# SparkJiao/llama-pipeline-parallel

Hardware: AMD Instinct MI355X
Metric: tokens/sec (whole node), LLaMA-65B PP=8 seq4096 at 1/2/4/8 MI355X (higher is better)
Workload: dtype bf16; 1 GPU; model=llama-65b, measured_model=llama-65b-shaped 10-layer slice (10/80 layers), global_batch=64, seq_len=4096, parallelism=pp1, num_layers=10, micro_batch_size=4, grad_accum_steps=16

## Files before the change

### lpp_amd/models/llama.py

```python

from __future__ import annotations

from typing import List, Optional

import torch
import torch.nn as nn

from ..config import ModelConfig
from ..layer_spec import LayerSpec
from .. import ops
from ..ops.linear import LPLinear, lp_linear


class RMSNorm(nn.Module):
    def __init__(self, hidden_size: int, eps: float = 1e-6):
        super().__init__()
        self.weight = nn.Parameter(torch.ones(hidden_size))
        self.variance_epsilon = eps

    def forward(self, x: torch.Tensor) -> torch.Tensor:
        return ops.rmsnorm(x, self.weight, self.variance_epsilon)


class KVCache:

    def __init__(self, batch: int, max_len: int, kv_heads: int, head_dim: int,
                 device, dtype):
        self.k = torch.zeros(batch, max_len, kv_heads, head_dim, device=device, dtype=dtype)
        self.v = torch.zeros_like(self.k)
        self.length = 0

    def append(self, k: torch.Tensor, v: torch.Tensor) -> int:
        S = k.shape[1]
        self.k[:, self.length : self.length + S] = k
        self.v[:, self.length : self.length + S] = v
        self.length += S
        return self.length


class SlotKVCache:

    def __init__(self, parent: "RaggedKVCache", slot: int):
        self.parent = parent
        self.slot = slot

    @property
    def k(self):
        return self.parent.k[self.slot : self.slot + 1]

    @property
    def v(self):
        return self.parent.v[self.slot : self.slot + 1]

    @property
    def length(self) -> int:
        return int(self.parent.lengths[self.slot])

    def append(self, k: torch.Tensor, v: torch.Tensor) -> int:
        S = k.shape[1]
        ln = self.length
        self.parent.k[self.slot, ln : ln + S] = k[0]
        self.parent.v[self.slot, ln : ln + S] = v[0]
        self.parent.lengths[self.slot] = ln + S
        return ln + S


class RaggedKVCache:

    per_row = True

    def __init__(self, slots: int, max_len: int, kv_heads: int, head_dim: int,
                 device, dtype):
        self.k = torch.zeros(slots, max_len, kv_heads, head_dim, device=device, dtype=dtype)
        self.v = torch.zeros_like(self.k)
        self.lengths = torch.zeros(slots, dtype=torch.long, device=device)

    def slot_view(self, slot: int) -> SlotKVCache:
        return SlotKVCache(self, slot)

    def free(self, slot: int) -> None:
        self.lengths[slot] = 0


class MultiSlotKVCache:

    def __init__(self, parent: RaggedKVCache, slots: torch.Tensor):
        self.parent = parent
        self.slots = slots
        self.length = 0

    def append(self, k: torch.Tensor, v: torch.Tensor) -> int:
        S = k.shape[1]
        self.parent.k[self.slots, self.length : self.length + S] = k
        self.parent.v[self.slots, self.length : self.length + S] = v
        self.length += S
        self.parent.lengths[self.slots] = self.length
        return self.length


class GatherKVCache:

    per_row = True

    def __init__(self, parent: RaggedKVCache, slots: torch.Tensor,
                 contiguous_range: Optional[tuple] = None,
                 total_hint: Optional[int] = None):
        self.parent = parent
        self.slots = slots
        self.range = contiguous_range
        self.total_hint = total_hint

    @property
    def k(self):
        return self.parent.k[self.slots]

    @property
    def v(self):
        return self.parent.v[self.slots]

    def kv_to(self, T: int):
        if self.range is not None:
            lo, hi = self.range
            return self.parent.k[lo:hi, :T], self.parent.v[lo:hi, :T]
        return self.parent.k[self.slots, :T], self.parent.v[self.slots, :T]

    @property
    def lengths(self) -> torch.Tensor:
        if self.range is not None:
            lo, hi = self.range
            return self.parent.lengths[lo:hi]
        return self.parent.lengths[self.slots]

    @property
    def rows(self) -> torch.Tensor:
        if getattr(self, "_rows", None) is None:
            if self.range is not None:
                lo, hi = self.range
                self._rows = torch.arange(lo, hi, device=self.parent.lengths.device)
            else:
                self._rows = self.slots
        return self._rows

    def append_one(self, k: torch.Tensor, v: torch.Tensor) -> torch.Tensor:
        lens = self.lengths
        if self.range is not None:
            lo, hi = self.range
            rows = torch.arange(lo, hi, device=lens.device)
        else:
            rows = self.slots
        self.parent.k[rows, lens] = k[:, 0]
        self.parent.v[rows, lens] = v[:, 0]
        new = lens + 1
        self.parent.lengths[rows] = new
        return new


class LlamaAttention(nn.Module):

    def __init__(self, cfg: ModelConfig):
        super().__init__()
        self.num_heads = cfg.num_heads
        self.num_kv_heads = cfg.kv_heads
        self.head_dim = cfg.head_dim
        self.hidden_size = cfg.hidden_size
        self.rope_theta = cfg.rope_theta
        self.max_seq_len = cfg.max_seq_len
        self.q_proj = LPLinear(cfg.hidden_size, self.num_heads * self.head_dim)
        self.k_proj = LPLinear(cfg.hidden_size, self.num_kv_heads * self.head_dim)
        self.v_proj = LPLinear(cfg.hidden_size, self.num_kv_heads * self.head_dim)
        self.o_proj = LPLinear(self.num_heads * self.head_dim, cfg.hidden_size)

    def forward(self, x: torch.Tensor, cache: Optional["KVCache"] = None) -> torch.Tensor:
        B, S, _ = x.shape
        q = self.q_proj(x).view(B, S, self.num_heads, self.head_dim)
        k = self.k_proj(x).view(B, S, self.num_kv_heads, self.head_dim)
        v = self.v_proj(x).view(B, S, self.num_kv_heads, self.head_dim)
        cos, sin = ops.build_rope_cache(
            self.max_seq_len, self.head_dim, self.rope_theta, x.device
        )
        if cache is not None and getattr(cache, "per_row", False):
            assert S == 1, "ragged cache is a single-token decode contract"
            tick = getattr(cache, "tick", None)
            if ops.decode_attention_hip_supported(q, self.num_kv_heads):
                parent = getattr(cache, "parent", cache)
                pos = getattr(tick, "pos", None)
                o = ops.decode_attention(
                    q, k, v, parent.k, parent.v, cos, sin,
                    pos if pos is not None else cache.lengths,
                    rows=cache.rows if parent is not cache else None,
                    lengths=parent.lengths,
                    max_len=getattr(cache, "total_hint", None))
                return self.o_proj(o.reshape(B, S, self.num_heads * self.head_dim))
            if tick is not None:
                q = ops.apply_rope_cs(q, tick.cos, tick.sin)
                k = ops.apply_rope_cs(k, tick.cos, tick.sin)
            else:
                lens = cache.lengths
                q = ops.apply_rope_positions(q, cos, sin, lens)
                k = ops.apply_rope_positions(k, cos, sin, lens)
            new_lens = cache.append_one(k, v)
            hint = getattr(cache, "total_hint", None)
            T = hint if hint is not None else int(new_lens.max())
            if hasattr(cache, "kv_to"):
                kc, vc = cache.kv_to(T)
            else:
                kc, vc = cache.k[:, :T], cache.v[:, :T]
            rep = self.num_heads // self.num_kv_heads
            qt = q.transpose(1, 2)
            kt = kc.transpose(1, 2)
            vt = vc.transpose(1, 2)
            if rep > 1:
                kt = kt.repeat_interleave(rep, dim=1)
                vt = vt.repeat_interleave(rep, dim=1)
            if tick is not None:
                mask = tick.mask
            else:
                mask = (torch.arange(T, device=x.device)[None, :]
                        < new_lens[:, None])[:, None, None, :]
            o = torch.nn.functional.scaled_dot_product_attention(
                qt, kt, vt, attn_mask=mask
            ).transpose(1, 2).contiguous()
            return self.o_proj(o.reshape(B, S, self.num_heads * self.head_dim))
        pos = cache.length if cache is not None else 0
        if (S == 1 and pos > 0 and isinstance(cache, KVCache)
                and ops.decode_attention_hip_supported(q, self.num_kv_heads)):
            o = ops.decode_attention(q, k, v, cache.k, cache.v, cos, sin, pos,
                                     max_len=pos + 1)
            cache.length = pos + 1
            return self.o_proj(o.reshape(B, S, self.num_heads * self.head_dim))
        q = ops.apply_rope(q, cos, sin, pos_offset=pos)
        k = ops.apply_rope(k, cos, sin, pos_offset=pos)
        if cache is None:
            o = ops.causal_attention(q, k, v)
        else:
            total = cache.append(k, v)
            if S == total:
                o = ops.causal_attention(q, k, v)
            else:
                kc = cache.k[:, :total]
                vc = cache.v[:, :total]
                rep = self.num_heads // self.num_kv_heads
                qt = q.transpose(1, 2)
                kt = kc.transpose(1, 2)
                vt = vc.transpose(1, 2)
                if rep > 1:
                    kt = kt.repeat_interleave(rep, dim=1)
                    vt = vt.repeat_interleave(rep, dim=1)
                mask = None
                if S > 1:
                    qpos = torch.arange(pos, total, device=x.device)
                    kpos = torch.arange(total, device=x.device)
                    mask = kpos[None, :] <= qpos[:, None]
                o = torch.nn.functional.scaled_dot_product_attention(
                    qt, kt, vt, attn_mask=mask
                ).transpose(1, 2).contiguous()
        return self.o_proj(o.reshape(B, S, self.num_heads * self.head_dim))


class LlamaMLP(nn.Module):
    def __init__(self, cfg: ModelConfig):
        super().__init__()
        self.gate_proj = LPLinear(cfg.hidden_size, cfg.intermediate_size)
        self.up_proj = LPLinear(cfg.hidden_size, cfg.intermediate_size)
        self.down_proj = LPLinear(cfg.intermediate_size, cfg.hidden_size)

    def forward(self, x: torch.Tensor) -> torch.Tensor:
        return self.down_proj(ops.swiglu(self.gate_proj(x), self.up_proj(x)))


class DecoderLayerPipe(nn.Module):

    def __init__(self, cfg: ModelConfig, activation_checkpointing: bool = False):
        super().__init__()
        self.self_attn = LlamaAttention(cfg)
        self.mlp = LlamaMLP(cfg)
        self.input_layernorm = RMSNorm(cfg.hidden_size, cfg.rms_norm_eps)
        self.post_attention_layernorm = RMSNorm(cfg.hidden_size, cfg.rms_norm_eps)
        self.activation_checkpointing = activation_checkpointing

    def _forward_impl(self, hidden: torch.Tensor,
                      cache: Optional[KVCache] = None) -> torch.Tensor:
        hidden = hidden + self.self_attn(self.input_layernorm(hidden), cache=cache)
        hidden = hidden + self.mlp(self.post_attention_layernorm(hidden))
        return hidden

    def forward(self, hidden: torch.Tensor,
                cache: Optional[KVCache] = None) -> torch.Tensor:
        if self.activation_checkpointing and self.training and hidden.requires_grad:
            return torch.utils.checkpoint.checkpoint(
                self._forward_impl, hidden, use_reentrant=False, preserve_rng_state=False
            )
        return self._forward_impl(hidden, cache=cache)

    @staticmethod
    def spec_param_count(cfg: ModelConfig, activation_checkpointing: bool = False) -> int:
        h, i = cfg.hidden_size, cfg.intermediate_size
        kv = cfg.kv_heads * cfg.head_dim
        return h * h * 2 + 2 * h * kv + 3 * h * i + 2 * h


class EmbeddingPipe(nn.Embedding):

    def __init__(self, vocab_size: int, hidden_size: int):
        super().__init__(vocab_size, hidden_size)

    def forward(self, input_ids: torch.Tensor) -> torch.Tensor:
        return super().forward(input_ids)

    @staticmethod
    def spec_param_count(vocab_size: int, hidden_size: int) -> int:
        return vocab_size * hidden_size


class NormPipe(RMSNorm):

    @staticmethod
    def spec_param_count(hidden_size: int, eps: float = 1e-6) -> int:
        return hidden_size


class LMHeadPipe(nn.Linear):

    def __init__(self, hidden_size: int, vocab_size: int):
        super().__init__(hidden_size, vocab_size, bias=False)

    def forward(self, x: torch.Tensor) -> torch.Tensor:
        return lp_linear(x, self.weight)

    @staticmethod
    def spec_param_count(hidden_size: int, vocab_size: int) -> int:
        return hidden_size * vocab_size


def loss_fn(logits: torch.Tensor, labels: torch.Tensor) -> torch.Tensor:
    return ops.shifted_cross_entropy(logits, labels)


def get_layers_from_config(
    cfg: ModelConfig, activation_checkpointing: bool = False,
    checkpoint_fn=None,
) -> List[LayerSpec]:
    if cfg.tie_word_embeddings:
        raise ValueError(
            "tie_word_embeddings=True is not supported: LLaMA checkpoints are "
            "untied and the reference (README.md:44-46) warns against tying "
            "under pipeline parallelism. Set it to False.")
    specs: List[LayerSpec] = [LayerSpec(EmbeddingPipe, cfg.vocab_size, cfg.hidden_size)]
    for i in range(cfg.num_layers):
        ck = checkpoint_fn(i) if checkpoint_fn is not None else activation_checkpointing
        specs.append(LayerSpec(DecoderLayerPipe, cfg, ck))
    specs.append(LayerSpec(NormPipe, cfg.hidden_size, cfg.rms_norm_eps))
    specs.append(LayerSpec(LMHeadPipe, cfg.hidden_size, cfg.vocab_size))
    return specs


@torch.no_grad()
def init_weights(module: nn.Module, cfg: ModelConfig, generator: Optional[torch.Generator] = None):
    std = cfg.initializer_range
    for m in module.modules():
        if isinstance(m, nn.Linear):
            m.weight.normal_(0.0, std, generator=generator)
            if m.bias is not None:
                m.bias.zero_()
        elif isinstance(m, nn.Embedding):
            m.weight.normal_(0.0, std, generator=generator)
        elif isinstance(m, RMSNorm):
            m.weight.fill_(1.0)


@torch.no_grad()
def deterministic_layer_init(layer: nn.Module, cfg: ModelConfig, seed: int, global_idx: int):
    g = torch.Generator().manual_seed(seed * 100003 + global_idx)
    std = cfg.initializer_range
    for name, p in sorted(layer.named_parameters()):
        if p.dim() >= 2:
            p.copy_(torch.empty(p.shape, dtype=torch.float32).normal_(0.0, std, generator=g).to(p.dtype))
        else:
            p.fill_(1.0) if "norm" in name or isinstance(layer, (RMSNorm,)) else p.zero_()
    for m in layer.modules():
        if isinstance(m, RMSNorm):
            m.weight.fill_(1.0)


def init_pipeline_weights(pipeline_module, cfg: ModelConfig, seed: int) -> None:
    for local_idx, layer in enumerate(pipeline_module.layers):
        deterministic_layer_init(layer, cfg, seed, pipeline_module.global_layer_index(local_idx))


def init_monolithic_weights(model: "LlamaForCausalLM", seed: int) -> None:
    for gidx, layer in enumerate(model.layers):
        deterministic_layer_init(layer, model.cfg, seed, gidx)


def layers_from_model(model: "LlamaForCausalLM") -> List[nn.Module]:
    return list(model.layers)


class LlamaForCausalLM(nn.Module):

    def __init__(self, cfg: ModelConfig, activation_checkpointing: bool = False):
        super().__init__()
        self.cfg = cfg
        self.layers = nn.ModuleList(
            [s.build() for s in get_layers_from_config(cfg, activation_checkpointing)]
        )

    def forward(self, input_ids: torch.Tensor) -> torch.Tensor:
        x = input_ids
        for layer in self.layers:
            x = layer(x)
        return x

    def compute_loss(self, input_ids: torch.Tensor, labels: torch.Tensor) -> torch.Tensor:
        return loss_fn(self.forward(input_ids), labels)

    @torch.no_grad()
    def generate(self, input_ids: torch.Tensor, max_new_tokens: int,
                 eos_token_id: Optional[int] = None,
                 temperature: float = 0.0,
                 generator: Optional[torch.Generator] = None) -> torch.Tensor:
        was_training = self.training
        self.eval()
        B, S0 = input_ids.shape
        dev = input_ids.device
        p = next(self.parameters())
        max_len = S0 + max_new_tokens
        caches = [
            KVCache(B, max_len, self.cfg.kv_heads, self.cfg.head_dim, dev, p.dtype)
            for _ in range(self.cfg.num_layers)
        ]

        def step(ids: torch.Tensor) -> torch.Tensor:
            x = ids
            li = 0
            for layer in self.layers:
                if isinstance(layer, DecoderLayerPipe):
                    x = layer(x, cache=caches[li])
                    li += 1
                else:
                    x = layer(x)
            return x[:, -1]

        out = input_ids
        logits = step(input_ids)
        finished = torch.zeros(B, dtype=torch.bool, device=dev)
        for _ in range(max_new_tokens):
            if temperature > 0:
                probs = torch.softmax(logits.float() / temperature, dim=-1)
                nxt = torch.multinomial(probs, 1, generator=generator).squeeze(-1)
            else:
                nxt = logits.argmax(dim=-1)
            if eos_token_id is not None:
                nxt = torch.where(finished, torch.full_like(nxt, eos_token_id), nxt)
                finished |= nxt == eos_token_id
            out = torch.cat([out, nxt[:, None]], dim=1)
            if eos_token_id is not None and bool(finished.all()):
                break
            logits = step(nxt[:, None])
        if was_training:
            self.train()
        return out
```

### lpp_amd/ops/__init__.py

```python

from __future__ import annotations

import os

import torch

_EXT = None
_EXT_ERR: str | None = "not loaded yet"


def _load_extension():
    global _EXT, _EXT_ERR
    if _EXT is not None:
        return _EXT
    try:
        from . import build as _build

        _EXT = _build.load_extension()
        _EXT_ERR = None
        if torch.cuda.is_available():
            _pin_wgrad_algos(_EXT)
    except Exception as e:
        _EXT = None
        _EXT_ERR = f"{type(e).__name__}: {e}"
    return _EXT


def _pin_wgrad_algos(ext) -> None:
    import json

    path = os.path.join(os.path.dirname(__file__), "wgrad_algos.json")
    if not os.path.exists(path):
        return
    try:
        data = json.load(open(path))
        for entry in data.get("shapes", []):
            ext.wgrad_set_algo(entry["T"], entry["in"], entry["out"], entry["index"],
                               entry.get("kind", 0))
    except Exception as e:
        import logging

        logging.getLogger(__name__).warning(
            "wgrad algo pinning skipped: %s", e)


def force_eager() -> bool:
    return os.environ.get("LPP_FORCE_EAGER", "0") == "1"


def extension():
    ext = _load_extension()
    if ext is None:
        raise RuntimeError(
            "lpp_amd HIP extension is required on GPU but failed to load: "
            f"{_EXT_ERR}. Build it with `python -m lpp_amd.ops.build` "
            "(or __graft_entry__.build())."
        )
    return ext


def use_hip(*tensors: torch.Tensor) -> bool:
    if force_eager():
        return False
    if not tensors or not tensors[0].is_cuda:
        return False
    return True


from .rmsnorm import rmsnorm
from .rope import (build_rope_cache, apply_rope, apply_rope_positions,
                   apply_rope_cs)
from .swiglu import swiglu
from .cross_entropy import shifted_cross_entropy
from .attention import (causal_attention, decode_attention,
                        decode_attention_ref, decode_attention_hip_supported)

__all__ = [
    "rmsnorm",
    "build_rope_cache",
    "apply_rope",
    "apply_rope_positions",
    "apply_rope_cs",
    "swiglu",
    "shifted_cross_entropy",
    "causal_attention",
    "decode_attention",
    "decode_attention_ref",
    "decode_attention_hip_supported",
    "extension",
    "use_hip",
    "force_eager",
]
```

### lpp_amd/ops/csrc/bindings.cpp

```cpp
#include <torch/extension.h>

#include <string>
#include <tuple>
#include <vector>

std::vector<at::Tensor> rmsnorm_fwd(at::Tensor x, at::Tensor weight, double eps);
std::vector<at::Tensor> rmsnorm_bwd(at::Tensor dy, at::Tensor x, at::Tensor weight,
                                    at::Tensor invrms);
at::Tensor rope_fwd(at::Tensor x, at::Tensor cos_t, at::Tensor sin_t, int64_t pos_offset);
at::Tensor rope_bwd(at::Tensor dy, at::Tensor cos_t, at::Tensor sin_t, int64_t pos_offset);
at::Tensor swiglu_fwd(at::Tensor gate, at::Tensor up);
std::vector<at::Tensor> swiglu_bwd(at::Tensor dy, at::Tensor gate, at::Tensor up);
std::vector<at::Tensor> cross_entropy_fwd(at::Tensor logits, at::Tensor labels);
at::Tensor cross_entropy_bwd(at::Tensor logits, at::Tensor labels, at::Tensor lse,
                             double scale);
std::vector<at::Tensor> attention_fwd(at::Tensor q, at::Tensor k, at::Tensor v);
std::vector<at::Tensor> attention_bwd(at::Tensor dO, at::Tensor q, at::Tensor k,
                                      at::Tensor v, at::Tensor o, at::Tensor lse2);
void attention_set_block_order(int64_t mode);
int64_t attention_get_block_order();
at::Tensor attention_block_order(int64_t kind, int64_t nblk, int64_t nheads, int64_t G,
                                 int64_t mode);
at::Tensor attention_lds_addresses(std::string pattern, int64_t shape, int64_t idx);
std::vector<double> attention_time_kernel(std::string kernel, at::Tensor dO, at::Tensor q,
                                          at::Tensor k, at::Tensor v, at::Tensor o,
                                          at::Tensor lse2, int64_t mode, int64_t G,
                                          int64_t warmup, int64_t reps);
at::Tensor attention_decode(at::Tensor q, at::Tensor k_new, at::Tensor v_new,
                            at::Tensor k_cache, at::Tensor v_cache, at::Tensor cos_t,
                            at::Tensor sin_t, c10::optional<at::Tensor> positions,
                            c10::optional<at::Tensor> rows,
                            c10::optional<at::Tensor> lengths, int64_t uniform_pos,
                            int64_t max_len, int64_t chunk);
int64_t attention_decode_chunk();
at::Tensor mfma_test_16x16x32(at::Tensor A, at::Tensor B);
void wgrad_f32_accum(at::Tensor x, at::Tensor dy, at::Tensor dw);
void wgrad_f32_accum_pre(at::Tensor xT, at::Tensor dyT, at::Tensor dw);
void wgrad_bf16d_pre(at::Tensor xT, at::Tensor dyT, at::Tensor out);
at::Tensor transpose2d(at::Tensor in);
void accum_bf16_f32(at::Tensor dst, at::Tensor src);
std::vector<std::tuple<int64_t, double, std::string>> wgrad_tune(int64_t T, int64_t in,
                                                                 int64_t out,
                                                                 int64_t reps,
                                                                 int64_t kind);
void wgrad_set_algo(int64_t T, int64_t in, int64_t out, int64_t index, int64_t kind);
std::tuple<int64_t, std::string> wgrad_current_algo(int64_t T, int64_t in, int64_t out,
                                                    int64_t kind);
at::Tensor mfma_test_32x32x16(at::Tensor A, at::Tensor B);
std::vector<at::Tensor> attn_tile_test_roundtrip(at::Tensor tile);
at::Tensor attn_tile_test_tr_fragments(at::Tensor tile, int64_t shape, int64_t nrows,
                                       int64_t buf);
at::Tensor attn_tile_test_pack_pair(at::Tensor x);
at::Tensor attn_tile_test_pack_frag16(at::Tensor x);
void fused_adamw(std::vector<at::Tensor> params, std::vector<at::Tensor> masters,
                 std::vector<at::Tensor> grads, std::vector<at::Tensor> exp_avg,
                 std::vector<at::Tensor> exp_avg_sq, double lr, double beta1, double beta2,
                 double eps, double weight_decay, double bias1, double bias2,
                 double grad_scale);

PYBIND11_MODULE(TORCH_EXTENSION_NAME, m) {
  m.doc() = "lpp_amd gfx950 (MI355X/CDNA4) kernels";
  m.def("rmsnorm_fwd", &rmsnorm_fwd, "RMSNorm forward (y, invrms)");
  m.def("rmsnorm_bwd", &rmsnorm_bwd, "RMSNorm backward (dx, dw)");
  m.def("rope_fwd", &rope_fwd, "RoPE forward");
  m.def("rope_bwd", &rope_bwd, "RoPE backward");
  m.def("swiglu_fwd", &swiglu_fwd, "SwiGLU forward");
  m.def("swiglu_bwd", &swiglu_bwd, "SwiGLU backward (dgate, dup)");
  m.def("cross_entropy_fwd", &cross_entropy_fwd, "fused CE forward (loss_sum, lse, count)");
  m.def("cross_entropy_bwd", &cross_entropy_bwd, "fused CE backward (dlogits)");
  m.def("fused_adamw", &fused_adamw, "fused mixed-precision AdamW");
  m.def("attention_fwd", &attention_fwd, "flash causal attention forward (O, LSE2)");
  m.def("attention_bwd", &attention_bwd, "flash causal attention backward (dQ, dK, dV)");
  m.def("attention_set_block_order", &attention_set_block_order,
        "attention block order: 0 = legacy, 1 = XCD-balanced heavy-first (default, "
        "LPP_ATTN_ORDER)", py::arg("mode"));
  m.def("attention_get_block_order", &attention_get_block_order, "current order mode");
  m.def("attention_block_order", &attention_block_order,
        "host: [n,2] int (blk, head) of linear block ids 0..n-1; kind 0 fwd/dQ, 1 dK/dV",
        py::arg("kind"), py::arg("nblk"), py::arg("nheads"), py::arg("G"), py::arg("mode"));
  m.def("attention_time_kernel", &attention_time_kernel,
        "hipEvent ms per launch of one attention kernel (fwd|dq|dkdv) under an explicit "
        "block order", py::arg("kernel"), py::arg("dO"), py::arg("q"), py::arg("k"),
        py::arg("v"), py::arg("o"), py::arg("lse2"), py::arg("mode"), py::arg("G") = 0,
        py::arg("warmup") = 3, py::arg("reps") = 20);
  m.def("attention_decode", &attention_decode,
        "fused single-token decode: RoPE + KV-cache write + GQA attention over keys 0..p of "
        "each row's cache row -> o [N,1,H,128]; chunk 0 = the compiled-in chunk size",
        py::arg("q"), py::arg("k_new"), py::arg("v_new"), py::arg("k_cache"),
        py::arg("v_cache"), py::arg("cos"), py::arg("sin"), py::arg("positions"),
        py::arg("rows"), py::arg("lengths"), py::arg("uniform_pos"), py::arg("max_len"),
        py::arg("chunk") = 0);
  m.def("attention_decode_chunk", &attention_decode_chunk,
        "keys per workgroup of attention_decode");
  m.def("wgrad_f32_accum", &wgrad_f32_accum, "dW_f32 += dY^T @ X (hipBLASLt, beta=1)");
  m.def("wgrad_f32_accum_pre", &wgrad_f32_accum_pre,
        "dW_f32 += dyT @ xT^T, pre-transposed k-contiguous operands (hipBLASLt, beta=1)");
  m.def("transpose2d", &transpose2d, "bf16/fp16 [R,C] -> [C,R] LDS-tiled transpose");
  m.def("wgrad_bf16d_pre", &wgrad_bf16d_pre,
        "bf16-D pre-transposed wgrad GEMM into a reusable scratch (beta 0)");
  m.def("accum_bf16_f32", &accum_bf16_f32, "dst_f32 += src_bf16 (vectorised)");
  m.def("wgrad_tune", &wgrad_tune,
        "exhaustive hipBLASLt solution sweep for a wgrad shape -> [(index, ms, name)]",
        py::arg("T"), py::arg("in_dim"), py::arg("out"), py::arg("reps"), py::arg("kind") = 0);
  m.def("wgrad_set_algo", &wgrad_set_algo, "pin a hipBLASLt solution index for a shape",
        py::arg("T"), py::arg("in_dim"), py::arg("out"), py::arg("index"), py::arg("kind") = 0);
  m.def("wgrad_current_algo", &wgrad_current_algo,
        "current (heuristic-picked) solution for a shape -> (index, name)",
        py::arg("T"), py::arg("in_dim"), py::arg("out"), py::arg("kind") = 0);
  m.def("mfma_test_16x16x32", &mfma_test_16x16x32, "MFMA layout validation");
  m.def("mfma_test_32x32x16", &mfma_test_32x32x16, "MFMA 32x32x16 layout validation");
  m.def("attn_tile_test_roundtrip", &attn_tile_test_roundtrip,
        "attn_tile.h dual-use image: int16 [64,128] -> (tile by row reads, transpose by "
        "transposed reads) from one LDS image");
  m.def("attn_tile_test_tr_fragments", &attn_tile_test_tr_fragments,
        "attn_tile.h transposed reads: int16 [64,128] -> int16 [16,64,8], the B-fragments "
        "of MFMA shape 32 (frag = dt*4+ks) or 16 (frag = dt*2+half) as the kernels read them",
        py::arg("tile"), py::arg("shape"), py::arg("nrows") = 64, py::arg("buf") = 0);
  m.def("attention_lds_addresses", &attention_lds_addresses,
        "host: int32 [64] per-lane LDS byte addresses of one access pattern (stage | row | "
        "tr) of MFMA shape 32 or 16", py::arg("pattern"), py::arg("shape"), py::arg("idx"));
  m.def("attn_tile_test_pack_pair", &attn_tile_test_pack_pair,
        "attn_tile.h pack_pair: fp32 [32,32] in C layout -> int32 [64,2,4] A-fragment words");
  m.def("attn_tile_test_pack_frag16", &attn_tile_test_pack_frag16,
        "attn_tile.h pack_frag16: fp32 [32,16] in C layout -> int32 [64,4] A-fragment words");
}
```

### lpp_amd/ops/csrc/rmsnorm.hip

```cpp
#include "common.h"

namespace lpp {

constexpr int BLOCK = 256;

template <typename T, int VEC>
__global__ void rmsnorm_fwd_kernel(const T* __restrict__ x, const float* __restrict__ w,
                                   T* __restrict__ y, float* __restrict__ invrms,
                                   int64_t n_rows, int H, float eps) {
  __shared__ float red[BLOCK / kWave];
  for (int64_t row = blockIdx.x; row < n_rows; row += gridDim.x) {
    const T* xr = x + row * H;
    T* yr = y + row * H;
    using PV = Pack<T, VEC>;
    float ss = 0.f;
    for (int i = threadIdx.x * VEC; i < H; i += BLOCK * VEC) {
      PV buf = *reinterpret_cast<const PV*>(xr + i);
#pragma unroll
      for (int v = 0; v < VEC; ++v) {
        float f = to_f32(buf.v[v]);
        ss += f * f;
      }
    }
    float total = block_reduce_sum<BLOCK>(ss, red);
    float inv = rsqrtf(total / (float)H + eps);
    if (threadIdx.x == 0) invrms[row] = inv;
    for (int i = threadIdx.x * VEC; i < H; i += BLOCK * VEC) {
      PV xin = *reinterpret_cast<const PV*>(xr + i);
      PV out;
#pragma unroll
      for (int v = 0; v < VEC; ++v)
        out.v[v] = from_f32<T>(to_f32(xin.v[v]) * inv * w[i + v]);
      *reinterpret_cast<PV*>(yr + i) = out;
    }
  }
}

template <typename T>
__global__ void rmsnorm_fwd_kernel_s(const T* __restrict__ x, const float* __restrict__ w,
                                     T* __restrict__ y, float* __restrict__ invrms,
                                     int64_t n_rows, int H, float eps) {
  __shared__ float red[BLOCK / kWave];
  for (int64_t row = blockIdx.x; row < n_rows; row += gridDim.x) {
    const T* xr = x + row * H;
    T* yr = y + row * H;
    float ss = 0.f;
    for (int i = threadIdx.x; i < H; i += BLOCK) {
      float f = to_f32(xr[i]);
      ss += f * f;
    }
    float total = block_reduce_sum<BLOCK>(ss, red);
    float inv = rsqrtf(total / (float)H + eps);
    if (threadIdx.x == 0) invrms[row] = inv;
    for (int i = threadIdx.x; i < H; i += BLOCK)
      yr[i] = from_f32<T>(to_f32(xr[i]) * inv * w[i]);
  }
}

template <typename T, int VEC, int N_IT>
__global__ void rmsnorm_bwd_kernel_v(const T* __restrict__ dy, const T* __restrict__ x,
                                     const float* __restrict__ w,
                                     const float* __restrict__ invrms, T* __restrict__ dx,
                                     float* __restrict__ dw_partial, int64_t n_rows,
                                     int H) {
  __shared__ float red[BLOCK / kWave];
  using PV = Pack<T, VEC>;
  alignas(16) float dwacc[N_IT][VEC];
  alignas(16) float wreg[N_IT][VEC];
#pragma unroll
  for (int it = 0; it < N_IT; ++it) {
    const int i = threadIdx.x * VEC + it * BLOCK * VEC;
    *reinterpret_cast<Pack<float, 4>*>(&wreg[it][0]) =
        *reinterpret_cast<const Pack<float, 4>*>(w + i);
    *reinterpret_cast<Pack<float, 4>*>(&wreg[it][4]) =
        *reinterpret_cast<const Pack<float, 4>*>(w + i + 4);
#pragma unroll
    for (int v = 0; v < VEC; ++v) dwacc[it][v] = 0.f;
  }

  for (int64_t row = blockIdx.x; row < n_rows; row += gridDim.x) {
    const T* dyr = dy + row * H;
    const T* xr = x + row * H;
    T* dxr = dx + row * H;
    const float inv = invrms[row];
    PV dybuf[N_IT], xbuf[N_IT];
    float dot = 0.f;
#pragma unroll
    for (int it = 0; it < N_IT; ++it) {
      const int i = threadIdx.x * VEC + it * BLOCK * VEC;
      dybuf[it] = *reinterpret_cast<const PV*>(dyr + i);
      xbuf[it] = *reinterpret_cast<const PV*>(xr + i);
#pragma unroll
      for (int v = 0; v < VEC; ++v)
        dot += to_f32(dybuf[it].v[v]) * wreg[it][v] * to_f32(xbuf[it].v[v]);
    }
    const float total = block_reduce_sum<BLOCK>(dot, red);
    const float k = total * inv * inv * inv / (float)H;
#pragma unroll
    for (int it = 0; it < N_IT; ++it) {
      const int i = threadIdx.x * VEC + it * BLOCK * VEC;
      PV out;
#pragma unroll
      for (int v = 0; v < VEC; ++v) {
        const float d = to_f32(dybuf[it].v[v]);
        const float xi = to_f32(xbuf[it].v[v]);
        out.v[v] = from_f32<T>(d * wreg[it][v] * inv - xi * k);
        dwacc[it][v] += d * xi * inv;
      }
      *reinterpret_cast<PV*>(dxr + i) = out;
    }
  }
  float* my = dw_partial + (int64_t)blockIdx.x * H;
#pragma unroll
  for (int it = 0; it < N_IT; ++it) {
    const int i = threadIdx.x * VEC + it * BLOCK * VEC;
    *reinterpret_cast<Pack<float, 4>*>(my + i) = *reinterpret_cast<Pack<float, 4>*>(&dwacc[it][0]);
    *reinterpret_cast<Pack<float, 4>*>(my + i + 4) = *reinterpret_cast<Pack<float, 4>*>(&dwacc[it][4]);
  }
}

template <typename T>
__global__ void rmsnorm_bwd_kernel(const T* __restrict__ dy, const T* __restrict__ x,
                                   const float* __restrict__ w,
                                   const float* __restrict__ invrms, T* __restrict__ dx,
                                   float* __restrict__ dw, int64_t n_rows, int H) {
  __shared__ float red[BLOCK / kWave];
  extern __shared__ __attribute__((aligned(16))) char smem[];
  float* dw_loc = reinterpret_cast<float*>(smem);
  for (int i = threadIdx.x; i < H; i += BLOCK) dw_loc[i] = 0.f;
  __syncthreads();

  for (int64_t row = blockIdx.x; row < n_rows; row += gridDim.x) {
    const T* dyr = dy + row * H;
    const T* xr = x + row * H;
    T* dxr = dx + row * H;
    const float inv = invrms[row];
    float dot = 0.f;
    for (int i = threadIdx.x; i < H; i += BLOCK) {
      float d = to_f32(dyr[i]);
      float xi = to_f32(xr[i]);
      dot += d * w[i] * xi;
      dw_loc[i] += d * xi * inv;
    }
    float total = block_reduce_sum<BLOCK>(dot, red);
    float k = total * inv * inv * inv / (float)H;
    for (int i = threadIdx.x; i < H; i += BLOCK) {
      float d = to_f32(dyr[i]);
      float xi = to_f32(xr[i]);
      dxr[i] = from_f32<T>(d * w[i] * inv - xi * k);
    }
  }
  __syncthreads();
  for (int i = threadIdx.x; i < H; i += BLOCK) atomicAdd(&dw[i], dw_loc[i]);
}

}

std::vector<at::Tensor> rmsnorm_fwd(at::Tensor x, at::Tensor weight, double eps) {
  TORCH_CHECK(x.is_cuda() && x.is_contiguous(), "rmsnorm_fwd: x must be contiguous on GPU");
  const int H = x.size(-1);
  const int64_t n_rows = x.numel() / H;
  auto y = at::empty_like(x);
  auto invrms = at::empty({n_rows}, x.options().dtype(at::kFloat));
  auto w32 = weight.to(at::kFloat).contiguous();
  auto stream = lpp::current_stream();
  const int grid = lpp::grid_for(n_rows, 1, 4096);
  LPP_DISPATCH_FLOAT(x.scalar_type(), "rmsnorm_fwd", [&] {
    constexpr int VEC = 16 / sizeof(scalar_t);
    if (H % VEC == 0) {
      hipLaunchKernelGGL((lpp::rmsnorm_fwd_kernel<scalar_t, VEC>), dim3(grid),
                         dim3(lpp::BLOCK), 0, stream, (const scalar_t*)x.data_ptr(),
                         w32.data_ptr<float>(), (scalar_t*)y.data_ptr(),
                         invrms.data_ptr<float>(), n_rows, H, (float)eps);
    } else {
      hipLaunchKernelGGL((lpp::rmsnorm_fwd_kernel_s<scalar_t>), dim3(grid),
                         dim3(lpp::BLOCK), 0, stream, (const scalar_t*)x.data_ptr(),
                         w32.data_ptr<float>(), (scalar_t*)y.data_ptr(),
                         invrms.data_ptr<float>(), n_rows, H, (float)eps);
    }
  });
  LPP_CHECK_HIP(hipGetLastError());
  return {y, invrms};
}

std::vector<at::Tensor> rmsnorm_bwd(at::Tensor dy, at::Tensor x, at::Tensor weight,
                                    at::Tensor invrms) {
  TORCH_CHECK(dy.is_cuda() && dy.is_contiguous() && x.is_contiguous());
  const int H = x.size(-1);
  const int64_t n_rows = x.numel() / H;
  auto dx = at::empty_like(x);
  auto dw32 = at::zeros({H}, x.options().dtype(at::kFloat));
  auto w32 = weight.to(at::kFloat).contiguous();
  auto stream = lpp::current_stream();
  LPP_DISPATCH_FLOAT(x.scalar_type(), "rmsnorm_bwd", [&] {
    constexpr int VEC = 16 / sizeof(scalar_t);
    const int n_it = H / (lpp::BLOCK * VEC);
    if (VEC == 8 && H % (lpp::BLOCK * VEC) == 0 && n_it >= 1 && n_it <= 4) {
      const int grid = lpp::grid_for(n_rows, 1, 2048);
      auto partial = at::empty({grid, H}, x.options().dtype(at::kFloat));
      auto launch = [&](auto kern) {
        hipLaunchKernelGGL(kern, dim3(grid), dim3(lpp::BLOCK), 0, stream,
                           (const scalar_t*)dy.data_ptr(), (const scalar_t*)x.data_ptr(),
                           w32.data_ptr<float>(), invrms.data_ptr<float>(),
                           (scalar_t*)dx.data_ptr(), partial.data_ptr<float>(), n_rows, H);
      };
      if (n_it == 1) launch(lpp::rmsnorm_bwd_kernel_v<scalar_t, VEC, 1>);
      else if (n_it == 2) launch(lpp::rmsnorm_bwd_kernel_v<scalar_t, VEC, 2>);
      else if (n_it == 3) launch(lpp::rmsnorm_bwd_kernel_v<scalar_t, VEC, 3>);
      else launch(lpp::rmsnorm_bwd_kernel_v<scalar_t, VEC, 4>);
      LPP_CHECK_HIP(hipGetLastError());
      at::sum_out(dw32, partial, {0});
    } else {
      const int grid = lpp::grid_for(n_rows, 1, 1024);
      const size_t lds = (size_t)H * sizeof(float);
      TORCH_CHECK(lds <= 160 * 1024 - 4096, "rmsnorm_bwd: H too large for LDS dw buffer");
      hipLaunchKernelGGL((lpp::rmsnorm_bwd_kernel<scalar_t>), dim3(grid), dim3(lpp::BLOCK),
                         lds, stream, (const scalar_t*)dy.data_ptr(),
                         (const scalar_t*)x.data_ptr(), w32.data_ptr<float>(),
                         invrms.data_ptr<float>(), (scalar_t*)dx.data_ptr(),
                         dw32.data_ptr<float>(), n_rows, H);
    }
  });
  LPP_CHECK_HIP(hipGetLastError());
  return {dx, dw32.to(weight.scalar_type())};
}
```

### lpp_amd/ops/csrc/rope.hip

```cpp
#include "common.h"

namespace lpp {

template <typename T, bool BWD>
__global__ void rope_kernel(const T* __restrict__ x, const float* __restrict__ cos_t,
                            const float* __restrict__ sin_t, T* __restrict__ y,
                            int64_t total_pairs4,
                            int S, int H, int D, int pos_offset) {
  const int half = D / 2;
  const int pair4_per_head = half / 4;
  for (int64_t idx = blockIdx.x * (int64_t)blockDim.x + threadIdx.x; idx < total_pairs4;
       idx += (int64_t)gridDim.x * blockDim.x) {
    const int p4 = idx % pair4_per_head;
    const int64_t bsh = idx / pair4_per_head;
    const int s = (int)((bsh / H) % S);
    const int d0 = p4 * 4;
    const int64_t base = bsh * D + d0;

    using P4 = Pack<T, 4>;
    P4 x1 = *reinterpret_cast<const P4*>(x + base);
    P4 x2 = *reinterpret_cast<const P4*>(x + base + half);
    P4 y1, y2;
    const float* cr = cos_t + (int64_t)(pos_offset + s) * half + d0;
    const float* sr = sin_t + (int64_t)(pos_offset + s) * half + d0;
#pragma unroll
    for (int k = 0; k < 4; ++k) {
      float c = cr[k];
      float sn = BWD ? -sr[k] : sr[k];
      float a = to_f32(x1.v[k]);
      float b = to_f32(x2.v[k]);
      y1.v[k] = from_f32<T>(a * c - b * sn);
      y2.v[k] = from_f32<T>(b * c + a * sn);
    }
    *reinterpret_cast<P4*>(y + base) = y1;
    *reinterpret_cast<P4*>(y + base + half) = y2;
  }
}

template <bool BWD>
at::Tensor rope_launch(at::Tensor x, at::Tensor cos_t, at::Tensor sin_t, int64_t pos_offset) {
  TORCH_CHECK(x.is_cuda() && x.is_contiguous() && x.dim() == 4, "rope: x must be [B,S,H,D]");
  const int B = x.size(0), S = x.size(1), H = x.size(2), D = x.size(3);
  TORCH_CHECK(D % 8 == 0, "rope: head_dim must be a multiple of 8");
  TORCH_CHECK(cos_t.is_contiguous() && sin_t.is_contiguous());
  TORCH_CHECK(cos_t.size(0) >= pos_offset + S, "rope cache too short");
  auto y = at::empty_like(x);
  const int64_t total = (int64_t)B * S * H * (D / 8);
  auto stream = lpp::current_stream();
  const int grid = lpp::grid_for(total, 256);
  LPP_DISPATCH_FLOAT(x.scalar_type(), "rope", [&] {
    hipLaunchKernelGGL((lpp::rope_kernel<scalar_t, BWD>), dim3(grid), dim3(256), 0, stream,
                       (const scalar_t*)x.data_ptr(), cos_t.data_ptr<float>(),
                       sin_t.data_ptr<float>(), (scalar_t*)y.data_ptr(), total, S, H, D,
                       (int)pos_offset);
  });
  LPP_CHECK_HIP(hipGetLastError());
  return y;
}

}

at::Tensor rope_fwd(at::Tensor x, at::Tensor cos_t, at::Tensor sin_t, int64_t pos_offset) {
  return lpp::rope_launch<false>(x, cos_t, sin_t, pos_offset);
}

at::Tensor rope_bwd(at::Tensor dy, at::Tensor cos_t, at::Tensor sin_t, int64_t pos_offset) {
  return lpp::rope_launch<true>(dy, cos_t, sin_t, pos_offset);
}
```

### lpp_amd/ops/csrc/swiglu.hip

```cpp
#include "common.h"

namespace lpp {

template <typename T, int VEC>
__global__ void swiglu_fwd_kernel(const T* __restrict__ g, const T* __restrict__ u,
                                  T* __restrict__ y, int64_t n_vec) {
  using PV = Pack<T, VEC>;
  for (int64_t i = blockIdx.x * (int64_t)blockDim.x + threadIdx.x; i < n_vec;
       i += (int64_t)gridDim.x * blockDim.x) {
    PV gp = reinterpret_cast<const PV*>(g)[i];
    PV up = reinterpret_cast<const PV*>(u)[i];
    PV yp;
#pragma unroll
    for (int v = 0; v < VEC; ++v) {
      float gf = to_f32(gp.v[v]);
      float s = 1.f / (1.f + __expf(-gf));
      yp.v[v] = from_f32<T>(gf * s * to_f32(up.v[v]));
    }
    reinterpret_cast<PV*>(y)[i] = yp;
  }
}

template <typename T, int VEC>
__global__ void swiglu_bwd_kernel(const T* __restrict__ dy, const T* __restrict__ g,
                                  const T* __restrict__ u, T* __restrict__ dg,
                                  T* __restrict__ du, int64_t n_vec) {
  using PV = Pack<T, VEC>;
  for (int64_t i = blockIdx.x * (int64_t)blockDim.x + threadIdx.x; i < n_vec;
       i += (int64_t)gridDim.x * blockDim.x) {
    PV dyp = reinterpret_cast<const PV*>(dy)[i];
    PV gp = reinterpret_cast<const PV*>(g)[i];
    PV up = reinterpret_cast<const PV*>(u)[i];
    PV dgp, dup;
#pragma unroll
    for (int v = 0; v < VEC; ++v) {
      float d = to_f32(dyp.v[v]);
      float gf = to_f32(gp.v[v]);
      float uf = to_f32(up.v[v]);
      float s = 1.f / (1.f + __expf(-gf));
      float silu = gf * s;
      float dsilu = s * (1.f + gf * (1.f - s));
      dgp.v[v] = from_f32<T>(d * uf * dsilu);
      dup.v[v] = from_f32<T>(d * silu);
    }
    reinterpret_cast<PV*>(dg)[i] = dgp;
    reinterpret_cast<PV*>(du)[i] = dup;
  }
}

}

at::Tensor swiglu_fwd(at::Tensor gate, at::Tensor up) {
  TORCH_CHECK(gate.is_cuda() && gate.is_contiguous() && up.is_contiguous());
  TORCH_CHECK(gate.sizes() == up.sizes() && gate.scalar_type() == up.scalar_type());
  auto y = at::empty_like(gate);
  const int64_t n = gate.numel();
  auto stream = lpp::current_stream();
  LPP_DISPATCH_FLOAT(gate.scalar_type(), "swiglu_fwd", [&] {
    constexpr int VEC = 16 / sizeof(scalar_t);
    TORCH_CHECK(n % VEC == 0, "swiglu: numel must be divisible by ", VEC);
    const int64_t n_vec = n / VEC;
    const int grid = lpp::grid_for(n_vec, 256);
    hipLaunchKernelGGL((lpp::swiglu_fwd_kernel<scalar_t, VEC>), dim3(grid), dim3(256), 0,
                       stream, (const scalar_t*)gate.data_ptr(),
                       (const scalar_t*)up.data_ptr(), (scalar_t*)y.data_ptr(), n_vec);
  });
  LPP_CHECK_HIP(hipGetLastError());
  return y;
}

std::vector<at::Tensor> swiglu_bwd(at::Tensor dy, at::Tensor gate, at::Tensor up) {
  TORCH_CHECK(dy.is_cuda() && dy.is_contiguous());
  auto dg = at::empty_like(gate);
  auto du = at::empty_like(up);
  const int64_t n = gate.numel();
  auto stream = lpp::current_stream();
  LPP_DISPATCH_FLOAT(gate.scalar_type(), "swiglu_bwd", [&] {
    constexpr int VEC = 16 / sizeof(scalar_t);
    const int64_t n_vec = n / VEC;
    const int grid = lpp::grid_for(n_vec, 256);
    hipLaunchKernelGGL((lpp::swiglu_bwd_kernel<scalar_t, VEC>), dim3(grid), dim3(256), 0,
                       stream, (const scalar_t*)dy.data_ptr(),
                       (const scalar_t*)gate.data_ptr(), (const scalar_t*)up.data_ptr(),
                       (scalar_t*)dg.data_ptr(), (scalar_t*)du.data_ptr(), n_vec);
  });
  LPP_CHECK_HIP(hipGetLastError());
  return {dg, du};
}
```

### lpp_amd/ops/csrc/transpose.hip

```cpp
#include "common.h"

namespace lpp {

constexpr int kTile = 64;
constexpr int kLdsStride = 66;

template <typename T>
__global__ __launch_bounds__(256) void transpose2d_kernel(
    const T* __restrict__ in, T* __restrict__ out, int R, int C) {
  __shared__ T tile[kTile * kLdsStride];

  const int c0 = blockIdx.x * kTile;
  const int r0 = blockIdx.y * kTile;

  const int tcp = threadIdx.x & 7;
  const int trow = threadIdx.x >> 3;
  const bool full = (r0 + kTile <= R) && (c0 + kTile <= C);
  if (full) {
#pragma unroll
    for (int i = 0; i < 2; ++i) {
      const int r = trow + 32 * i;
      const Pack<T, 8> p = *reinterpret_cast<const Pack<T, 8>*>(
          in + (int64_t)(r0 + r) * C + c0 + tcp * 8);
#pragma unroll
      for (int e = 0; e < 8; ++e) tile[r * kLdsStride + tcp * 8 + e] = p.v[e];
    }
  } else {
#pragma unroll
    for (int i = 0; i < 2; ++i) {
      const int r = trow + 32 * i;
#pragma unroll
      for (int e = 0; e < 8; ++e) {
        const int rr = r0 + r, cc = c0 + tcp * 8 + e;
        tile[r * kLdsStride + tcp * 8 + e] =
            (rr < R && cc < C) ? in[(int64_t)rr * C + cc] : T{};
      }
    }
  }
  __syncthreads();

  if (full) {
#pragma unroll
    for (int i = 0; i < 2; ++i) {
      const int c = trow + 32 * i;
      Pack<T, 8> p;
#pragma unroll
      for (int e = 0; e < 8; ++e) p.v[e] = tile[(tcp * 8 + e) * kLdsStride + c];
      *reinterpret_cast<Pack<T, 8>*>(out + (int64_t)(c0 + c) * R + r0 + tcp * 8) = p;
    }
  } else {
#pragma unroll
    for (int i = 0; i < 2; ++i) {
      const int c = trow + 32 * i;
#pragma unroll
      for (int e = 0; e < 8; ++e) {
        const int cc = c0 + c, rr = r0 + tcp * 8 + e;
        if (cc < C && rr < R)
          out[(int64_t)cc * R + rr] = tile[(tcp * 8 + e) * kLdsStride + c];
      }
    }
  }
}


typedef __attribute__((ext_vector_type(8))) short bf16x8_t;
typedef __attribute__((ext_vector_type(2))) int int2v_t;

__device__ __forceinline__ int t2swz(int d, int r) {
  return (d * 64 + (r ^ ((((d >> 3) ^ d) & 7) << 3))) * 2;
}

__global__ __launch_bounds__(256) void transpose2d_v2_kernel(
    const short* __restrict__ in, short* __restrict__ out, int R, int C) {
  __shared__ __attribute__((aligned(16))) char img[128 * 64 * 2];

  const int tid = threadIdx.x;
  const int wid = tid >> 6;
  const int lane = tid & 63;
  const int st_r = (lane >> 4) & 3;
  const int st_c = 8 * (lane & 15);

  const int r0 = blockIdx.y * 64;
  const int c0 = blockIdx.x * 128;

#pragma unroll
  for (int pass = 0; pass < 4; ++pass) {
    const int r = 4 * wid + 16 * pass + st_r;
    const bf16x8_t v = *reinterpret_cast<const bf16x8_t*>(
        in + (int64_t)(r0 + r) * C + c0 + st_c);
    int dw[4];
#pragma unroll
    for (int k = 0; k < 4; ++k) dw[k] = reinterpret_cast<const int*>(&v)[k];
    {
      int t0 = __shfl_xor(dw[(st_r & 1) ^ 1], 16);
      int t1 = __shfl_xor(dw[((st_r & 1) ^ 1) | 2], 16);
      if (st_r & 1) { dw[0] = t0; dw[2] = t1; } else { dw[1] = t0; dw[3] = t1; }
    }
    {
      int lo = (st_r & 2) ? 0 : 2;
      int t0 = __shfl_xor(dw[lo], 32);
      int t1 = __shfl_xor(dw[lo + 1], 32);
      dw[lo] = t0; dw[lo + 1] = t1;
    }
    const int rq = 4 * wid + 16 * pass;
    const int d0 = st_c + 2 * st_r;
#pragma unroll
    for (int e = 0; e < 2; ++e) {
      const int d = d0 + e;
      unsigned w01 = e ? (((unsigned)dw[0] >> 16) | ((unsigned)dw[1] & 0xffff0000u))
                       : (((unsigned)dw[0] & 0xffffu) | ((unsigned)dw[1] << 16));
      unsigned w23 = e ? (((unsigned)dw[2] >> 16) | ((unsigned)dw[3] & 0xffff0000u))
                       : (((unsigned)dw[2] & 0xffffu) | ((unsigned)dw[3] << 16));
      int2v_t pair = {(int)w01, (int)w23};
      *reinterpret_cast<int2v_t*>(img + t2swz(d, rq)) = pair;
    }
  }
  __syncthreads();

#pragma unroll
  for (int pass = 0; pass < 4; ++pass) {
    const int d = 32 * pass + (tid >> 3);
    const int p = tid & 7;
    const bf16x8_t v = *reinterpret_cast<const bf16x8_t*>(img + t2swz(d, 8 * p));
    *reinterpret_cast<bf16x8_t*>(out + (int64_t)(c0 + d) * R + r0 + 8 * p) = v;
  }
}

at::Tensor transpose2d(at::Tensor in) {
  TORCH_CHECK(in.is_cuda() && in.dim() == 2 && in.is_contiguous());
  TORCH_CHECK(in.scalar_type() == at::kBFloat16 || in.scalar_type() == at::kHalf,
              "transpose2d: bf16/fp16 only");
  const int R = (int)in.size(0), C = (int)in.size(1);
  auto out = at::empty({C, R}, in.options());
  auto stream = current_stream();
  if (in.scalar_type() == at::kBFloat16 && R % 64 == 0 && C % 128 == 0) {
    dim3 grid(C / 128, R / 64);
    hipLaunchKernelGGL(transpose2d_v2_kernel, grid, dim3(256), 0, stream,
                       reinterpret_cast<const short*>(in.data_ptr()),
                       reinterpret_cast<short*>(out.data_ptr()), R, C);
    LPP_CHECK_HIP(hipGetLastError());
    return out;
  }
  dim3 grid((C + kTile - 1) / kTile, (R + kTile - 1) / kTile);
  if (in.scalar_type() == at::kBFloat16) {
    hipLaunchKernelGGL(transpose2d_kernel<__hip_bfloat16>, grid, dim3(256), 0, stream,
                       reinterpret_cast<const __hip_bfloat16*>(in.data_ptr()),
                       reinterpret_cast<__hip_bfloat16*>(out.data_ptr()), R, C);
  } else {
    hipLaunchKernelGGL(transpose2d_kernel<__half>, grid, dim3(256), 0, stream,
                       reinterpret_cast<const __half*>(in.data_ptr()),
                       reinterpret_cast<__half*>(out.data_ptr()), R, C);
  }
  LPP_CHECK_HIP(hipGetLastError());
  return out;
}

}

at::Tensor transpose2d(at::Tensor in) { return lpp::transpose2d(in); }
```

### lpp_amd/ops/linear.py

```python

from __future__ import annotations

import os

import torch
import torch.nn.functional as F

from . import extension, force_eager


class _XTCache:

    __slots__ = ("x", "xT")

    def __init__(self):
        self.x = None
        self.xT = None

    def get(self, ext, x2: torch.Tensor) -> torch.Tensor:
        if (self.x is not None and self.x.data_ptr() == x2.data_ptr()
                and self.x.shape == x2.shape and self.x.dtype == x2.dtype):
            return self.xT
        xT = ext.transpose2d(x2)
        self.x = x2
        self.xT = xT
        return xT

    def clear(self):
        self.x = None
        self.xT = None


_xt_cache = _XTCache()


def _wgrad_pre_enabled() -> bool:
    return os.environ.get("LPP_WGRAD_PRE", "1") == "1"


def _wgrad_bf16d_enabled() -> bool:
    return os.environ.get("LPP_WGRAD_BF16D", "1") == "1"


def _dgrad_wt_enabled() -> bool:
    return os.environ.get("LPP_DGRAD_WT", "1") == "1"


def _weight_t(ext, weight: torch.nn.Parameter) -> torch.Tensor:
    wt = getattr(weight, "_wt", None)
    if wt is None:
        wt = ext.transpose2d(weight.data)
        weight._wt = wt
    return wt


def invalidate_weight_transposes(module: torch.nn.Module) -> None:
    for p in module.parameters():
        if hasattr(p, "_wt"):
            p._wt = None


class _LinearWgradF32(torch.autograd.Function):
    @staticmethod
    def forward(ctx, x: torch.Tensor, weight: torch.nn.Parameter):
        ctx.save_for_backward(x, weight)
        ctx.main_grad = weight.main_grad
        return F.linear(x, weight)

    @staticmethod
    def backward(ctx, dy: torch.Tensor):
        x, weight = ctx.saved_tensors
        dy = dy.contiguous()
        ext = extension()
        if _dgrad_wt_enabled():
            dx = dy @ _weight_t(ext, weight).t()
        else:
            dx = dy @ weight
        x2 = x.reshape(-1, x.shape[-1]).contiguous()
        dy2 = dy.reshape(-1, dy.shape[-1])
        if _wgrad_pre_enabled():
            xT = _xt_cache.get(ext, x2)
            dyT = ext.transpose2d(dy2)
            if _wgrad_bf16d_enabled():
                ext.accum_bf16_f32(ctx.main_grad.view(-1),
                                   torch.matmul(dyT, xT.t()).view(-1))
            else:
                ext.wgrad_f32_accum_pre(xT, dyT, ctx.main_grad)
        else:
            ext.wgrad_f32_accum(x2, dy2, ctx.main_grad)
        cb = getattr(weight, "_on_accumulate", None)
        if cb is not None:
            cb(weight)
        return dx, None


def lp_linear(x: torch.Tensor, weight: torch.nn.Parameter) -> torch.Tensor:
    if (
        x.is_cuda
        and x.dtype is torch.bfloat16
        and torch.is_grad_enabled()
        and weight.requires_grad
        and hasattr(weight, "main_grad")
        and not force_eager()
    ):
        return _LinearWgradF32.apply(x, weight)
    return F.linear(x, weight)


class LPLinear(torch.nn.Linear):

    def __init__(self, in_features: int, out_features: int, bias: bool = False):
        assert not bias, "LLaMA projections are bias-free"
        super().__init__(in_features, out_features, bias=False)

    def forward(self, x: torch.Tensor) -> torch.Tensor:
        return lp_linear(x, self.weight)
```

### lpp_amd/ops/rmsnorm.py

```python

from __future__ import annotations

import torch

from . import use_hip, extension


def rmsnorm_ref(x: torch.Tensor, weight: torch.Tensor, eps: float) -> torch.Tensor:
    xf = x.float()
    inv = torch.rsqrt(xf.pow(2).mean(-1, keepdim=True) + eps)
    return (xf * inv * weight.float()).to(x.dtype)


class _RMSNormHIP(torch.autograd.Function):
    @staticmethod
    def forward(ctx, x, weight, eps):
        ext = extension()
        y, invrms = ext.rmsnorm_fwd(x, weight, eps)
        ctx.save_for_backward(x, weight, invrms)
        return y

    @staticmethod
    def backward(ctx, dy):
        x, weight, invrms = ctx.saved_tensors
        ext = extension()
        dx, dw = ext.rmsnorm_bwd(dy.contiguous(), x, weight, invrms)
        return dx, dw, None


def rmsnorm(x: torch.Tensor, weight: torch.Tensor, eps: float = 1e-6) -> torch.Tensor:
    if use_hip(x):
        return _RMSNormHIP.apply(x.contiguous(), weight, eps)
    return rmsnorm_ref(x, weight, eps)
```

### lpp_amd/ops/rope.py

```python

from __future__ import annotations

from typing import Tuple

import torch

from . import use_hip, extension

_CACHE: dict = {}


def build_rope_cache(
    seq_len: int, head_dim: int, theta: float, device, dtype=torch.float32
) -> Tuple[torch.Tensor, torch.Tensor]:
    key = (seq_len, head_dim, theta, str(device))
    hit = _CACHE.get(key)
    if hit is not None:
        return hit
    inv_freq = 1.0 / (
        theta ** (torch.arange(0, head_dim, 2, device=device, dtype=torch.float32) / head_dim)
    )
    t = torch.arange(seq_len, device=device, dtype=torch.float32)
    freqs = torch.outer(t, inv_freq)
    out = (freqs.cos().contiguous(), freqs.sin().contiguous())
    _CACHE[key] = out
    return out


def apply_rope_ref(
    x: torch.Tensor, cos: torch.Tensor, sin: torch.Tensor, pos_offset: int = 0
) -> torch.Tensor:
    B, S, H, D = x.shape
    c = cos[pos_offset : pos_offset + S].view(1, S, 1, D // 2).to(torch.float32)
    s = sin[pos_offset : pos_offset + S].view(1, S, 1, D // 2).to(torch.float32)
    xf = x.float()
    x1, x2 = xf[..., : D // 2], xf[..., D // 2 :]
    out = torch.cat((x1 * c - x2 * s, x2 * c + x1 * s), dim=-1)
    return out.to(x.dtype)


class _RopeHIP(torch.autograd.Function):
    @staticmethod
    def forward(ctx, x, cos, sin, pos_offset):
        ext = extension()
        y = ext.rope_fwd(x, cos, sin, pos_offset)
        ctx.save_for_backward(cos, sin)
        ctx.pos_offset = pos_offset
        return y

    @staticmethod
    def backward(ctx, dy):
        cos, sin = ctx.saved_tensors
        ext = extension()
        dx = ext.rope_bwd(dy.contiguous(), cos, sin, ctx.pos_offset)
        return dx, None, None, None


def apply_rope(
    x: torch.Tensor, cos: torch.Tensor, sin: torch.Tensor, pos_offset: int = 0
) -> torch.Tensor:
    if use_hip(x):
        return _RopeHIP.apply(x.contiguous(), cos, sin, pos_offset)
    return apply_rope_ref(x, cos, sin, pos_offset)


@torch.no_grad()
def apply_rope_cs(x: torch.Tensor, c: torch.Tensor, s: torch.Tensor) -> torch.Tensor:
    D = x.shape[-1]
    xf = x.float()
    x1, x2 = xf[..., : D // 2], xf[..., D // 2 :]
    return torch.cat((x1 * c - x2 * s, x2 * c + x1 * s), dim=-1).to(x.dtype)


@torch.no_grad()
def apply_rope_positions(
    x: torch.Tensor, cos: torch.Tensor, sin: torch.Tensor, positions: torch.Tensor
) -> torch.Tensor:
    N, S, H, D = x.shape
    assert S == 1, "positions variant is a single-token decode contract"
    c = cos[positions].view(N, 1, 1, D // 2).to(torch.float32)
    s = sin[positions].view(N, 1, 1, D // 2).to(torch.float32)
    return apply_rope_cs(x, c, s)
```

### lpp_amd/ops/swiglu.py

```python

from __future__ import annotations

import torch

from . import use_hip, extension


def swiglu_ref(gate: torch.Tensor, up: torch.Tensor) -> torch.Tensor:
    gf = gate.float()
    return (gf * torch.sigmoid(gf) * up.float()).to(gate.dtype)


class _SwiGLUHIP(torch.autograd.Function):
    @staticmethod
    def forward(ctx, gate, up):
        ext = extension()
        y = ext.swiglu_fwd(gate, up)
        ctx.save_for_backward(gate, up)
        return y

    @staticmethod
    def backward(ctx, dy):
        gate, up = ctx.saved_tensors
        ext = extension()
        dgate, dup = ext.swiglu_bwd(dy.contiguous(), gate, up)
        return dgate, dup


def swiglu(gate: torch.Tensor, up: torch.Tensor) -> torch.Tensor:
    if use_hip(gate):
        return _SwiGLUHIP.apply(gate.contiguous(), up.contiguous())
    return swiglu_ref(gate, up)
```

Baseline: 23940 tokens/s.

## Fuse backward gradient transposes into elementwise kernels and hand off to wgrad

The backward kernels for RMSNorm, RoPE and SwiGLU now also write the transposed gradient image, and a small pointer-keyed cache hands it to the linear layer's weight-gradient path so it can skip its own transpose2d launch. The decoder layer routes through a forked RMSNorm whose backward sums the q/k/v (or gate/up) partial gradients and the residual gradient in one fused kernel, replacing the separate autograd adds. The dw reduction in the non-vectorized kernel moves from atomics to per-block partials. In exchange the code gains a fragile data_ptr-keyed cache and extra transpose writes from the elementwise kernels, and the summation order and bf16 rounding of the gradients change.

```diff
diff --git a/lpp_amd/models/llama.py b/lpp_amd/models/llama.py
--- a/lpp_amd/models/llama.py
+++ b/lpp_amd/models/llama.py
@@ -170,11 +170,15 @@
         self.v_proj = LPLinear(cfg.hidden_size, self.num_kv_heads * self.head_dim)
         self.o_proj = LPLinear(self.num_heads * self.head_dim, cfg.hidden_size)
 
-    def forward(self, x: torch.Tensor, cache: Optional["KVCache"] = None) -> torch.Tensor:
+    def forward(self, x: torch.Tensor, cache: Optional["KVCache"] = None,
+                x_k: Optional[torch.Tensor] = None,
+                x_v: Optional[torch.Tensor] = None) -> torch.Tensor:
         B, S, _ = x.shape
         q = self.q_proj(x).view(B, S, self.num_heads, self.head_dim)
-        k = self.k_proj(x).view(B, S, self.num_kv_heads, self.head_dim)
-        v = self.v_proj(x).view(B, S, self.num_kv_heads, self.head_dim)
+        k = self.k_proj(x if x_k is None else x_k).view(
+            B, S, self.num_kv_heads, self.head_dim)
+        v = self.v_proj(x if x_v is None else x_v).view(
+            B, S, self.num_kv_heads, self.head_dim)
         cos, sin = ops.build_rope_cache(
             self.max_seq_len, self.head_dim, self.rope_theta, x.device
         )
@@ -264,8 +268,9 @@
         self.up_proj = LPLinear(cfg.hidden_size, cfg.intermediate_size)
         self.down_proj = LPLinear(cfg.intermediate_size, cfg.hidden_size)
 
-    def forward(self, x: torch.Tensor) -> torch.Tensor:
-        return self.down_proj(ops.swiglu(self.gate_proj(x), self.up_proj(x)))
+    def forward(self, x: torch.Tensor, x_up: Optional[torch.Tensor] = None) -> torch.Tensor:
+        return self.down_proj(ops.swiglu(
+            self.gate_proj(x), self.up_proj(x if x_up is None else x_up)))
 
 
 class DecoderLayerPipe(nn.Module):
@@ -280,8 +285,23 @@
 
     def _forward_impl(self, hidden: torch.Tensor,
                       cache: Optional[KVCache] = None) -> torch.Tensor:
+        if cache is None and ops.rmsnorm_fork_applies(hidden) and (
+                hidden.requires_grad or self.input_layernorm.weight.requires_grad):
+            return self._forward_fork(hidden)
         hidden = hidden + self.self_attn(self.input_layernorm(hidden), cache=cache)
         hidden = hidden + self.mlp(self.post_attention_layernorm(hidden))
+        return hidden
+
+    def _forward_fork(self, hidden: torch.Tensor) -> torch.Tensor:
+        ln = self.input_layernorm
+        want_t = getattr(hidden, "_lpp_decoder_out", False)
+        hidden, xq, xk, xv = ops.rmsnorm_fork(
+            hidden, ln.weight, ln.variance_epsilon, 3, want_t)
+        hidden = hidden + self.self_attn(xq, x_k=xk, x_v=xv)
+        ln = self.post_attention_layernorm
+        hidden, xg, xu = ops.rmsnorm_fork(hidden, ln.weight, ln.variance_epsilon, 2, True)
+        hidden = hidden + self.mlp(xg, x_up=xu)
+        hidden._lpp_decoder_out = True
         return hidden
 
     def forward(self, hidden: torch.Tensor,
diff --git a/lpp_amd/ops/__init__.py b/lpp_amd/ops/__init__.py
--- a/lpp_amd/ops/__init__.py
+++ b/lpp_amd/ops/__init__.py
@@ -67,7 +67,7 @@
     return True
 
 
-from .rmsnorm import rmsnorm
+from .rmsnorm import rmsnorm, rmsnorm_fork, rmsnorm_fork_applies
 from .rope import (build_rope_cache, apply_rope, apply_rope_positions,
                    apply_rope_cs)
 from .swiglu import swiglu
@@ -77,6 +77,8 @@
 
 __all__ = [
     "rmsnorm",
+    "rmsnorm_fork",
+    "rmsnorm_fork_applies",
     "build_rope_cache",
     "apply_rope",
     "apply_rope_positions",
diff --git a/lpp_amd/ops/csrc/bindings.cpp b/lpp_amd/ops/csrc/bindings.cpp
--- a/lpp_amd/ops/csrc/bindings.cpp
+++ b/lpp_amd/ops/csrc/bindings.cpp
@@ -7,10 +7,16 @@
 std::vector<at::Tensor> rmsnorm_fwd(at::Tensor x, at::Tensor weight, double eps);
 std::vector<at::Tensor> rmsnorm_bwd(at::Tensor dy, at::Tensor x, at::Tensor weight,
                                     at::Tensor invrms);
+std::vector<at::Tensor> rmsnorm_bwd_fused(std::vector<at::Tensor> dys, at::Tensor x,
+                                          at::Tensor weight, at::Tensor invrms,
+                                          c10::optional<at::Tensor> dres, bool want_t);
 at::Tensor rope_fwd(at::Tensor x, at::Tensor cos_t, at::Tensor sin_t, int64_t pos_offset);
 at::Tensor rope_bwd(at::Tensor dy, at::Tensor cos_t, at::Tensor sin_t, int64_t pos_offset);
+std::vector<at::Tensor> rope_bwd_t(at::Tensor dy, at::Tensor cos_t, at::Tensor sin_t,
+                                   int64_t pos_offset);
 at::Tensor swiglu_fwd(at::Tensor gate, at::Tensor up);
 std::vector<at::Tensor> swiglu_bwd(at::Tensor dy, at::Tensor gate, at::Tensor up);
+std::vector<at::Tensor> swiglu_bwd_t(at::Tensor dy, at::Tensor gate, at::Tensor up);
 std::vector<at::Tensor> cross_entropy_fwd(at::Tensor logits, at::Tensor labels);
 at::Tensor cross_entropy_bwd(at::Tensor logits, at::Tensor labels, at::Tensor lse,
                              double scale);
@@ -62,10 +68,21 @@
   m.doc() = "lpp_amd gfx950 (MI355X/CDNA4) kernels";
   m.def("rmsnorm_fwd", &rmsnorm_fwd, "RMSNorm forward (y, invrms)");
   m.def("rmsnorm_bwd", &rmsnorm_bwd, "RMSNorm backward (dx, dw)");
+  m.def("rmsnorm_bwd_fused", &rmsnorm_bwd_fused,
+        "RMSNorm backward with the gradient adds fused: sums 1..3 partial dy (bf16 rounding "
+        "after each add), adds dres to the rounded dx -> (dx_total, dw, dxT or empty)",
+        py::arg("dys"), py::arg("x"), py::arg("weight"), py::arg("invrms"),
+        py::arg("dres") = py::none(), py::arg("want_t") = false);
   m.def("rope_fwd", &rope_fwd, "RoPE forward");
   m.def("rope_bwd", &rope_bwd, "RoPE backward");
+  m.def("rope_bwd_t", &rope_bwd_t,
+        "RoPE backward that also writes dx^T [H*D, B*S] when aligned (D = 128, B*S % 64 == "
+        "0, bf16): (dx, dxT), else (dx,)");
   m.def("swiglu_fwd", &swiglu_fwd, "SwiGLU forward");
   m.def("swiglu_bwd", &swiglu_bwd, "SwiGLU backward (dgate, dup)");
+  m.def("swiglu_bwd_t", &swiglu_bwd_t,
+        "SwiGLU backward that also writes dgate^T, dup^T [I, T] when aligned (T % 64 == 0, "
+        "I % 128 == 0, bf16): (dgate, dup, dgateT, dupT), else (dgate, dup)");
   m.def("cross_entropy_fwd", &cross_entropy_fwd, "fused CE forward (loss_sum, lse, count)");
   m.def("cross_entropy_bwd", &cross_entropy_bwd, "fused CE backward (dlogits)");
   m.def("fused_adamw", &fused_adamw, "fused mixed-precision AdamW");
diff --git a/lpp_amd/ops/csrc/rmsnorm.hip b/lpp_amd/ops/csrc/rmsnorm.hip
--- a/lpp_amd/ops/csrc/rmsnorm.hip
+++ b/lpp_amd/ops/csrc/rmsnorm.hip
@@ -57,8 +57,17 @@
   }
 }
 
-template <typename T, int VEC, int N_IT>
-__global__ void rmsnorm_bwd_kernel_v(const T* __restrict__ dy, const T* __restrict__ x,
+template <typename T, int NDY>
+__device__ __forceinline__ T sum_partials(T a, T b, T c) {
+  if (NDY >= 2) a = from_f32<T>(to_f32(a) + to_f32(b));
+  if (NDY >= 3) a = from_f32<T>(to_f32(a) + to_f32(c));
+  return a;
+}
+
+template <typename T, int VEC, int N_IT, int NDY, bool HAS_RES>
+__global__ __launch_bounds__(BLOCK) void rmsnorm_bwd_kernel_v(const T* __restrict__ dy, const T* __restrict__ dy1,
+                                     const T* __restrict__ dy2, const T* __restrict__ dres,
+                                     const T* __restrict__ x,
                                      const float* __restrict__ w,
                                      const float* __restrict__ invrms, T* __restrict__ dx,
                                      float* __restrict__ dw_partial, int64_t n_rows,
@@ -89,6 +98,14 @@
     for (int it = 0; it < N_IT; ++it) {
       const int i = threadIdx.x * VEC + it * BLOCK * VEC;
       dybuf[it] = *reinterpret_cast<const PV*>(dyr + i);
+      if (NDY >= 2) {
+        PV p1 = *reinterpret_cast<const PV*>(dy1 + row * H + i);
+        PV p2 = p1;
+        if (NDY >= 3) p2 = *reinterpret_cast<const PV*>(dy2 + row * H + i);
+#pragma unroll
+        for (int v = 0; v < VEC; ++v)
+          dybuf[it].v[v] = sum_partials<T, NDY>(dybuf[it].v[v], p1.v[v], p2.v[v]);
+      }
       xbuf[it] = *reinterpret_cast<const PV*>(xr + i);
 #pragma unroll
       for (int v = 0; v < VEC; ++v)
@@ -100,11 +117,14 @@
     for (int it = 0; it < N_IT; ++it) {
       const int i = threadIdx.x * VEC + it * BLOCK * VEC;
       PV out;
+      PV rp;
+      if (HAS_RES) rp = *reinterpret_cast<const PV*>(dres + row * H + i);
 #pragma unroll
       for (int v = 0; v < VEC; ++v) {
         const float d = to_f32(dybuf[it].v[v]);
         const float xi = to_f32(xbuf[it].v[v]);
         out.v[v] = from_f32<T>(d * wreg[it][v] * inv - xi * k);
+        if (HAS_RES) out.v[v] = from_f32<T>(to_f32(out.v[v]) + to_f32(rp.v[v]));
         dwacc[it][v] += d * xi * inv;
       }
       *reinterpret_cast<PV*>(dxr + i) = out;
@@ -119,11 +139,14 @@
   }
 }
 
-template <typename T>
-__global__ void rmsnorm_bwd_kernel(const T* __restrict__ dy, const T* __restrict__ x,
+template <typename T, int NDY, bool HAS_RES>
+__global__ void rmsnorm_bwd_kernel(const T* __restrict__ dy, const T* __restrict__ dy1,
+                                   const T* __restrict__ dy2, const T* __restrict__ dres,
+                                   const T* __restrict__ x,
                                    const float* __restrict__ w,
                                    const float* __restrict__ invrms, T* __restrict__ dx,
-                                   float* __restrict__ dw, int64_t n_rows, int H) {
+                                   float* __restrict__ dw_partial, int64_t n_rows,
+                                   int H) {
   __shared__ float red[BLOCK / kWave];
   extern __shared__ __attribute__((aligned(16))) char smem[];
   float* dw_loc = reinterpret_cast<float*>(smem);
@@ -137,7 +160,8 @@
     const float inv = invrms[row];
     float dot = 0.f;
     for (int i = threadIdx.x; i < H; i += BLOCK) {
-      float d = to_f32(dyr[i]);
+      float d = to_f32(sum_partials<T, NDY>(dyr[i], NDY >= 2 ? dy1[row * H + i] : dyr[i],
+                                            NDY >= 3 ? dy2[row * H + i] : dyr[i]));
       float xi = to_f32(xr[i]);
       dot += d * w[i] * xi;
       dw_loc[i] += d * xi * inv;
@@ -145,13 +169,17 @@
     float total = block_reduce_sum<BLOCK>(dot, red);
     float k = total * inv * inv * inv / (float)H;
     for (int i = threadIdx.x; i < H; i += BLOCK) {
-      float d = to_f32(dyr[i]);
+      float d = to_f32(sum_partials<T, NDY>(dyr[i], NDY >= 2 ? dy1[row * H + i] : dyr[i],
+                                            NDY >= 3 ? dy2[row * H + i] : dyr[i]));
       float xi = to_f32(xr[i]);
-      dxr[i] = from_f32<T>(d * w[i] * inv - xi * k);
+      T o = from_f32<T>(d * w[i] * inv - xi * k);
+      if (HAS_RES) o = from_f32<T>(to_f32(o) + to_f32(dres[row * H + i]));
+      dxr[i] = o;
     }
   }
   __syncthreads();
-  for (int i = threadIdx.x; i < H; i += BLOCK) atomicAdd(&dw[i], dw_loc[i]);
+  float* my = dw_partial + (int64_t)blockIdx.x * H;
+  for (int i = threadIdx.x; i < H; i += BLOCK) my[i] = dw_loc[i];
 }
 
 }
@@ -183,44 +211,87 @@
   return {y, invrms};
 }
 
+namespace lpp {
+
+static std::vector<at::Tensor> rmsnorm_bwd_launch(const std::vector<at::Tensor>& dys,
+                                                  at::Tensor x, at::Tensor weight,
+                                                  at::Tensor invrms,
+                                                  const c10::optional<at::Tensor>& dres) {
+  const int H = x.size(-1);
+  const int64_t n_rows = x.numel() / H;
+  auto dx = at::empty_like(x);
+  auto dw32 = at::empty({H}, x.options().dtype(at::kFloat));
+  auto w32 = weight.to(at::kFloat).contiguous();
+  auto stream = current_stream();
+  const int ndy = (int)dys.size();
+  const bool has_res = dres.has_value();
+  LPP_DISPATCH_FLOAT(x.scalar_type(), "rmsnorm_bwd", [&] {
+    constexpr int VEC = 16 / sizeof(scalar_t);
+    const scalar_t* p0 = (const scalar_t*)dys[0].data_ptr();
+    const scalar_t* p1 = ndy >= 2 ? (const scalar_t*)dys[1].data_ptr() : p0;
+    const scalar_t* p2 = ndy >= 3 ? (const scalar_t*)dys[2].data_ptr() : p0;
+    const scalar_t* pr = has_res ? (const scalar_t*)dres->data_ptr() : p0;
+    const int n_it = H / (BLOCK * VEC);
+    const bool vec = VEC == 8 && H % (BLOCK * VEC) == 0 && n_it >= 1 && n_it <= 4;
+    const int grid = grid_for(n_rows, 1, vec ? 2048 : 1024);
+    auto partial = at::empty({grid, H}, x.options().dtype(at::kFloat));
+    const size_t lds = vec ? 0 : (size_t)H * sizeof(float);
+    TORCH_CHECK(lds <= 160 * 1024 - 4096, "rmsnorm_bwd: H too large for LDS dw buffer");
+    auto launch = [&](auto kern) {
+      hipLaunchKernelGGL(kern, dim3(grid), dim3(BLOCK), lds, stream, p0, p1, p2, pr,
+                         (const scalar_t*)x.data_ptr(), w32.data_ptr<float>(),
+                         invrms.data_ptr<float>(), (scalar_t*)dx.data_ptr(),
+                         partial.data_ptr<float>(), n_rows, H);
+    };
+    auto pick = [&](auto ndy_c, auto res_c) {
+      constexpr int NDY = decltype(ndy_c)::value;
+      constexpr bool RES = decltype(res_c)::value;
+      if (!vec) launch(rmsnorm_bwd_kernel<scalar_t, NDY, RES>);
+      else if (n_it == 1) launch(rmsnorm_bwd_kernel_v<scalar_t, VEC, 1, NDY, RES>);
+      else if (n_it == 2) launch(rmsnorm_bwd_kernel_v<scalar_t, VEC, 2, NDY, RES>);
+      else if (n_it == 3) launch(rmsnorm_bwd_kernel_v<scalar_t, VEC, 3, NDY, RES>);
+      else launch(rmsnorm_bwd_kernel_v<scalar_t, VEC, 4, NDY, RES>);
+    };
+    auto pick_res = [&](auto ndy_c) {
+      if (has_res) pick(ndy_c, std::true_type{});
+      else pick(ndy_c, std::false_type{});
+    };
+    if (ndy == 1) pick_res(std::integral_constant<int, 1>{});
+    else if (ndy == 2) pick_res(std::integral_constant<int, 2>{});
+    else pick_res(std::integral_constant<int, 3>{});
+    LPP_CHECK_HIP(hipGetLastError());
+    at::sum_out(dw32, partial, {0});
+  });
+  return {dx, dw32.to(weight.scalar_type())};
+}
+
+}
+
 std::vector<at::Tensor> rmsnorm_bwd(at::Tensor dy, at::Tensor x, at::Tensor weight,
                                     at::Tensor invrms) {
   TORCH_CHECK(dy.is_cuda() && dy.is_contiguous() && x.is_contiguous());
-  const int H = x.size(-1);
-  const int64_t n_rows = x.numel() / H;
-  auto dx = at::empty_like(x);
-  auto dw32 = at::zeros({H}, x.options().dtype(at::kFloat));
-  auto w32 = weight.to(at::kFloat).contiguous();
-  auto stream = lpp::current_stream();
-  LPP_DISPATCH_FLOAT(x.scalar_type(), "rmsnorm_bwd", [&] {
-    constexpr int VEC = 16 / sizeof(scalar_t);
-    const int n_it = H / (lpp::BLOCK * VEC);
-    if (VEC == 8 && H % (lpp::BLOCK * VEC) == 0 && n_it >= 1 && n_it <= 4) {
-      const int grid = lpp::grid_for(n_rows, 1, 2048);
-      auto partial = at::empty({grid, H}, x.options().dtype(at::kFloat));
-      auto launch = [&](auto kern) {
-        hipLaunchKernelGGL(kern, dim3(grid), dim3(lpp::BLOCK), 0, stream,
-                           (const scalar_t*)dy.data_ptr(), (const scalar_t*)x.data_ptr(),
-                           w32.data_ptr<float>(), invrms.data_ptr<float>(),
-                           (scalar_t*)dx.data_ptr(), partial.data_ptr<float>(), n_rows, H);
-      };
-      if (n_it == 1) launch(lpp::rmsnorm_bwd_kernel_v<scalar_t, VEC, 1>);
-      else if (n_it == 2) launch(lpp::rmsnorm_bwd_kernel_v<scalar_t, VEC, 2>);
-      else if (n_it == 3) launch(lpp::rmsnorm_bwd_kernel_v<scalar_t, VEC, 3>);
-      else launch(lpp::rmsnorm_bwd_kernel_v<scalar_t, VEC, 4>);
-      LPP_CHECK_HIP(hipGetLastError());
-      at::sum_out(dw32, partial, {0});
-    } else {
-      const int grid = lpp::grid_for(n_rows, 1, 1024);
-      const size_t lds = (size_t)H * sizeof(float);
-      TORCH_CHECK(lds <= 160 * 1024 - 4096, "rmsnorm_bwd: H too large for LDS dw buffer");
-      hipLaunchKernelGGL((lpp::rmsnorm_bwd_kernel<scalar_t>), dim3(grid), dim3(lpp::BLOCK),
-                         lds, stream, (const scalar_t*)dy.data_ptr(),
-                         (const scalar_t*)x.data_ptr(), w32.data_ptr<float>(),
-                         invrms.data_ptr<float>(), (scalar_t*)dx.data_ptr(),
-                         dw32.data_ptr<float>(), n_rows, H);
-    }
-  });
-  LPP_CHECK_HIP(hipGetLastError());
-  return {dx, dw32.to(weight.scalar_type())};
-}
+  return lpp::rmsnorm_bwd_launch({dy}, x, weight, invrms, c10::nullopt);
+}
+
+at::Tensor transpose2d(at::Tensor in);
+
+std::vector<at::Tensor> rmsnorm_bwd_fused(std::vector<at::Tensor> dys, at::Tensor x,
+                                          at::Tensor weight, at::Tensor invrms,
+                                          c10::optional<at::Tensor> dres, bool want_t) {
+  TORCH_CHECK(!dys.empty() && dys.size() <= 3, "rmsnorm_bwd_fused: 1..3 partial gradients");
+  TORCH_CHECK(x.is_cuda() && x.is_contiguous());
+  auto check = [&](const at::Tensor& t, const char* what) {
+    TORCH_CHECK(t.is_cuda() && t.is_contiguous() && t.scalar_type() == x.scalar_type() &&
+                    t.numel() == x.numel() && t.size(-1) == x.size(-1),
+                "rmsnorm_bwd_fused: ", what, " must match x (contiguous, same dtype/shape)");
+  };
+  for (const auto& t : dys) check(t, "dys");
+  if (dres.has_value()) check(*dres, "dres");
+  auto out = lpp::rmsnorm_bwd_launch(dys, x, weight, invrms, dres);
+  const int64_t H = x.size(-1), rows = x.numel() / H;
+  if (want_t && x.scalar_type() == at::kBFloat16 && rows % 64 == 0 && H % 128 == 0)
+    out.push_back(transpose2d(out[0].view({rows, H})));
+  else
+    out.push_back(at::empty({0}, x.options()));
+  return out;
+}
diff --git a/lpp_amd/ops/csrc/rope.hip b/lpp_amd/ops/csrc/rope.hip
--- a/lpp_amd/ops/csrc/rope.hip
+++ b/lpp_amd/ops/csrc/rope.hip
@@ -1,4 +1,5 @@
 #include "common.h"
+#include "transpose_tile.h"
 
 namespace lpp {
 
@@ -37,6 +38,51 @@
   }
 }
 
+__global__ __launch_bounds__(256) void rope_bwd_t_kernel(
+    const __hip_bfloat16* __restrict__ x, const float* __restrict__ cos_t,
+    const float* __restrict__ sin_t, __hip_bfloat16* __restrict__ y,
+    short* __restrict__ yT, int T, int S, int C , int pos_offset) {
+  __shared__ __attribute__((aligned(16))) char img[kTTImgBytes];
+  using T_ = __hip_bfloat16;
+  using PV = Pack<T_, 8>;
+  constexpr int half = 64;
+
+  const int r0 = blockIdx.y * 64;
+  const int c0 = blockIdx.x * 128;
+  const int col = tt_col();
+  const bool first = col < half;
+  const int d0 = col & (half - 1);
+
+#pragma unroll
+  for (int pass = 0; pass < 4; ++pass) {
+    const int row = r0 + tt_row(pass);
+    const int s = row % S;
+    const int64_t off = (int64_t)row * C + c0 + col;
+    PV own = *reinterpret_cast<const PV*>(x + off);
+    PV oth;
+#pragma unroll
+    for (int k = 0; k < 4; ++k)
+      reinterpret_cast<int*>(&oth)[k] = __shfl_xor(reinterpret_cast<const int*>(&own)[k], 8);
+    const float* cr = cos_t + (int64_t)(pos_offset + s) * half + d0;
+    const float* sr = sin_t + (int64_t)(pos_offset + s) * half + d0;
+    PV out;
+#pragma unroll
+    for (int k = 0; k < 8; ++k) {
+      float c = cr[k];
+      float sn = -sr[k];
+      float a = to_f32(first ? own.v[k] : oth.v[k]);
+      float b = to_f32(first ? oth.v[k] : own.v[k]);
+      T_ y1 = from_f32<T_>(a * c - b * sn);
+      T_ y2 = from_f32<T_>(b * c + a * sn);
+      out.v[k] = first ? y1 : y2;
+    }
+    *reinterpret_cast<PV*>(y + off) = out;
+    tt_stage(img, *reinterpret_cast<const bf16x8_t*>(&out), pass);
+  }
+  __syncthreads();
+  tt_store(img, yT, T, r0, c0);
+}
+
 template <bool BWD>
 at::Tensor rope_launch(at::Tensor x, at::Tensor cos_t, at::Tensor sin_t, int64_t pos_offset) {
   TORCH_CHECK(x.is_cuda() && x.is_contiguous() && x.dim() == 4, "rope: x must be [B,S,H,D]");
@@ -67,3 +113,28 @@
 at::Tensor rope_bwd(at::Tensor dy, at::Tensor cos_t, at::Tensor sin_t, int64_t pos_offset) {
   return lpp::rope_launch<true>(dy, cos_t, sin_t, pos_offset);
 }
+
+std::vector<at::Tensor> rope_bwd_t(at::Tensor dy, at::Tensor cos_t, at::Tensor sin_t,
+                                   int64_t pos_offset) {
+  TORCH_CHECK(dy.is_cuda() && dy.is_contiguous() && dy.dim() == 4,
+              "rope: x must be [B,S,H,D]");
+  const int64_t B = dy.size(0), S = dy.size(1), H = dy.size(2), D = dy.size(3);
+  const int64_t T = B * S, C = H * D;
+  if (dy.scalar_type() != at::kBFloat16 || D != 128 || T == 0 || T % 64 != 0 ||
+      T / 64 > 65535 || T > INT32_MAX || C > INT32_MAX)
+    return {lpp::rope_launch<true>(dy, cos_t, sin_t, pos_offset)};
+  TORCH_CHECK(cos_t.is_contiguous() && sin_t.is_contiguous());
+  TORCH_CHECK(cos_t.scalar_type() == at::kFloat && sin_t.scalar_type() == at::kFloat);
+  TORCH_CHECK(cos_t.dim() == 2 && cos_t.size(1) == D / 2 && sin_t.sizes() == cos_t.sizes(),
+              "rope: cos/sin must be [Smax, D/2]");
+  TORCH_CHECK(pos_offset >= 0 && cos_t.size(0) >= pos_offset + S, "rope cache too short");
+  auto dx = at::empty_like(dy);
+  auto dxT = at::empty({C, T}, dy.options());
+  dim3 grid((unsigned)H, (unsigned)(T / 64));
+  hipLaunchKernelGGL(lpp::rope_bwd_t_kernel, grid, dim3(256), 0, lpp::current_stream(),
+                     (const __hip_bfloat16*)dy.data_ptr(), cos_t.data_ptr<float>(),
+                     sin_t.data_ptr<float>(), (__hip_bfloat16*)dx.data_ptr(),
+                     (short*)dxT.data_ptr(), (int)T, (int)S, (int)C, (int)pos_offset);
+  LPP_CHECK_HIP(hipGetLastError());
+  return {dx, dxT};
+}
diff --git a/lpp_amd/ops/csrc/swiglu.hip b/lpp_amd/ops/csrc/swiglu.hip
--- a/lpp_amd/ops/csrc/swiglu.hip
+++ b/lpp_amd/ops/csrc/swiglu.hip
@@ -1,4 +1,5 @@
 #include "common.h"
+#include "transpose_tile.h"
 
 namespace lpp {
 
@@ -48,6 +49,46 @@
   }
 }
 
+__global__ __launch_bounds__(256) void swiglu_bwd_t_kernel(
+    const __hip_bfloat16* __restrict__ dy, const __hip_bfloat16* __restrict__ g,
+    const __hip_bfloat16* __restrict__ u, __hip_bfloat16* __restrict__ dg,
+    __hip_bfloat16* __restrict__ du, short* __restrict__ dgT, short* __restrict__ duT,
+    int T, int I) {
+  __shared__ __attribute__((aligned(16))) char img[2][kTTImgBytes];
+  using T_ = __hip_bfloat16;
+  using PV = Pack<T_, 8>;
+
+  const int r0 = blockIdx.y * 64;
+  const int c0 = blockIdx.x * 128;
+
+#pragma unroll
+  for (int pass = 0; pass < 4; ++pass) {
+    const int64_t off = (int64_t)(r0 + tt_row(pass)) * I + c0 + tt_col();
+    PV dyp = *reinterpret_cast<const PV*>(dy + off);
+    PV gp = *reinterpret_cast<const PV*>(g + off);
+    PV up = *reinterpret_cast<const PV*>(u + off);
+    PV dgp, dup;
+#pragma unroll
+    for (int v = 0; v < 8; ++v) {
+      float d = to_f32(dyp.v[v]);
+      float gf = to_f32(gp.v[v]);
+      float uf = to_f32(up.v[v]);
+      float s = 1.f / (1.f + __expf(-gf));
+      float silu = gf * s;
+      float dsilu = s * (1.f + gf * (1.f - s));
+      dgp.v[v] = from_f32<T_>(d * uf * dsilu);
+      dup.v[v] = from_f32<T_>(d * silu);
+    }
+    *reinterpret_cast<PV*>(dg + off) = dgp;
+    *reinterpret_cast<PV*>(du + off) = dup;
+    tt_stage(img[0], *reinterpret_cast<const bf16x8_t*>(&dgp), pass);
+    tt_stage(img[1], *reinterpret_cast<const bf16x8_t*>(&dup), pass);
+  }
+  __syncthreads();
+  tt_store(img[0], dgT, T, r0, c0);
+  tt_store(img[1], duT, T, r0, c0);
+}
+
 }
 
 at::Tensor swiglu_fwd(at::Tensor gate, at::Tensor up) {
@@ -87,3 +128,29 @@
   LPP_CHECK_HIP(hipGetLastError());
   return {dg, du};
 }
+
+std::vector<at::Tensor> swiglu_bwd_t(at::Tensor dy, at::Tensor gate, at::Tensor up) {
+  TORCH_CHECK(dy.is_cuda() && dy.is_contiguous() && gate.is_contiguous() &&
+              up.is_contiguous());
+  TORCH_CHECK(dy.sizes() == gate.sizes() && gate.sizes() == up.sizes() &&
+              dy.scalar_type() == gate.scalar_type() &&
+              gate.scalar_type() == up.scalar_type());
+  const int64_t I = gate.dim() >= 1 ? gate.size(-1) : 0;
+  const int64_t T = I > 0 ? gate.numel() / I : 0;
+  if (gate.scalar_type() != at::kBFloat16 || T == 0 || T % 64 != 0 || I % 128 != 0 ||
+      T / 64 > 65535 || T > INT32_MAX || I > INT32_MAX)
+    return swiglu_bwd(dy, gate, up);
+  auto dg = at::empty_like(gate);
+  auto du = at::empty_like(up);
+  auto dgT = at::empty({I, T}, gate.options());
+  auto duT = at::empty({I, T}, gate.options());
+  dim3 grid((unsigned)(I / 128), (unsigned)(T / 64));
+  hipLaunchKernelGGL(lpp::swiglu_bwd_t_kernel, grid, dim3(256), 0, lpp::current_stream(),
+                     (const __hip_bfloat16*)dy.data_ptr(),
+                     (const __hip_bfloat16*)gate.data_ptr(),
+                     (const __hip_bfloat16*)up.data_ptr(), (__hip_bfloat16*)dg.data_ptr(),
+                     (__hip_bfloat16*)du.data_ptr(), (short*)dgT.data_ptr(),
+                     (short*)duT.data_ptr(), (int)T, (int)I);
+  LPP_CHECK_HIP(hipGetLastError());
+  return {dg, du, dgT, duT};
+}
diff --git a/lpp_amd/ops/csrc/transpose.hip b/lpp_amd/ops/csrc/transpose.hip
--- a/lpp_amd/ops/csrc/transpose.hip
+++ b/lpp_amd/ops/csrc/transpose.hip
@@ -1,4 +1,5 @@
 #include "common.h"
+#include "transpose_tile.h"
 
 namespace lpp {
 
@@ -63,67 +64,21 @@
 }
 
 
-typedef __attribute__((ext_vector_type(8))) short bf16x8_t;
-typedef __attribute__((ext_vector_type(2))) int int2v_t;
-
-__device__ __forceinline__ int t2swz(int d, int r) {
-  return (d * 64 + (r ^ ((((d >> 3) ^ d) & 7) << 3))) * 2;
-}
-
 __global__ __launch_bounds__(256) void transpose2d_v2_kernel(
     const short* __restrict__ in, short* __restrict__ out, int R, int C) {
-  __shared__ __attribute__((aligned(16))) char img[128 * 64 * 2];
-
-  const int tid = threadIdx.x;
-  const int wid = tid >> 6;
-  const int lane = tid & 63;
-  const int st_r = (lane >> 4) & 3;
-  const int st_c = 8 * (lane & 15);
+  __shared__ __attribute__((aligned(16))) char img[kTTImgBytes];
 
   const int r0 = blockIdx.y * 64;
   const int c0 = blockIdx.x * 128;
 
 #pragma unroll
   for (int pass = 0; pass < 4; ++pass) {
-    const int r = 4 * wid + 16 * pass + st_r;
     const bf16x8_t v = *reinterpret_cast<const bf16x8_t*>(
-        in + (int64_t)(r0 + r) * C + c0 + st_c);
-    int dw[4];
-#pragma unroll
-    for (int k = 0; k < 4; ++k) dw[k] = reinterpret_cast<const int*>(&v)[k];
-    {
-      int t0 = __shfl_xor(dw[(st_r & 1) ^ 1], 16);
-      int t1 = __shfl_xor(dw[((st_r & 1) ^ 1) | 2], 16);
-      if (st_r & 1) { dw[0] = t0; dw[2] = t1; } else { dw[1] = t0; dw[3] = t1; }
-    }
-    {
-      int lo = (st_r & 2) ? 0 : 2;
-      int t0 = __shfl_xor(dw[lo], 32);
-      int t1 = __shfl_xor(dw[lo + 1], 32);
-      dw[lo] = t0; dw[lo + 1] = t1;
-    }
-    const int rq = 4 * wid + 16 * pass;
-    const int d0 = st_c + 2 * st_r;
-#pragma unroll
-    for (int e = 0; e < 2; ++e) {
-      const int d = d0 + e;
-      unsigned w01 = e ? (((unsigned)dw[0] >> 16) | ((unsigned)dw[1] & 0xffff0000u))
-                       : (((unsigned)dw[0] & 0xffffu) | ((unsigned)dw[1] << 16));
-      unsigned w23 = e ? (((unsigned)dw[2] >> 16) | ((unsigned)dw[3] & 0xffff0000u))
-                       : (((unsigned)dw[2] & 0xffffu) | ((unsigned)dw[3] << 16));
-      int2v_t pair = {(int)w01, (int)w23};
-      *reinterpret_cast<int2v_t*>(img + t2swz(d, rq)) = pair;
-    }
+        in + (int64_t)(r0 + tt_row(pass)) * C + c0 + tt_col());
+    tt_stage(img, v, pass);
   }
   __syncthreads();
-
-#pragma unroll
-  for (int pass = 0; pass < 4; ++pass) {
-    const int d = 32 * pass + (tid >> 3);
-    const int p = tid & 7;
-    const bf16x8_t v = *reinterpret_cast<const bf16x8_t*>(img + t2swz(d, 8 * p));
-    *reinterpret_cast<bf16x8_t*>(out + (int64_t)(c0 + d) * R + r0 + 8 * p) = v;
-  }
+  tt_store(img, out, R, r0, c0);
 }
 
 at::Tensor transpose2d(at::Tensor in) {
diff --git a/lpp_amd/ops/csrc/transpose_tile.h b/lpp_amd/ops/csrc/transpose_tile.h
--- /dev/null
+++ b/lpp_amd/ops/csrc/transpose_tile.h
@@ -0,0 +1,71 @@
+#pragma once
+
+#include <hip/hip_runtime.h>
+
+#include <cstdint>
+
+namespace lpp {
+
+typedef __attribute__((ext_vector_type(8))) short bf16x8_t;
+typedef __attribute__((ext_vector_type(2))) int int2v_t;
+
+constexpr int kTTRows = 64;
+constexpr int kTTCols = 128;
+constexpr int kTTImgBytes = kTTRows * kTTCols * 2;
+
+__device__ __forceinline__ int tt_swz(int d, int r) {
+  return (d * 64 + (r ^ ((((d >> 3) ^ d) & 7) << 3))) * 2;
+}
+
+__device__ __forceinline__ int tt_row(int pass) {
+  const int wid = threadIdx.x >> 6, lane = threadIdx.x & 63;
+  return 4 * wid + 16 * pass + ((lane >> 4) & 3);
+}
+__device__ __forceinline__ int tt_col() { return 8 * (threadIdx.x & 15); }
+
+__device__ __forceinline__ void tt_stage(char* img, bf16x8_t v, int pass) {
+  const int wid = threadIdx.x >> 6;
+  const int lane = threadIdx.x & 63;
+  const int st_r = (lane >> 4) & 3;
+  const int st_c = 8 * (lane & 15);
+  int dw[4];
+#pragma unroll
+  for (int k = 0; k < 4; ++k) dw[k] = reinterpret_cast<const int*>(&v)[k];
+  {
+    int t0 = __shfl_xor(dw[(st_r & 1) ^ 1], 16);
+    int t1 = __shfl_xor(dw[((st_r & 1) ^ 1) | 2], 16);
+    if (st_r & 1) { dw[0] = t0; dw[2] = t1; } else { dw[1] = t0; dw[3] = t1; }
+  }
+  {
+    int lo = (st_r & 2) ? 0 : 2;
+    int t0 = __shfl_xor(dw[lo], 32);
+    int t1 = __shfl_xor(dw[lo + 1], 32);
+    dw[lo] = t0; dw[lo + 1] = t1;
+  }
+  const int rq = 4 * wid + 16 * pass;
+  const int d0 = st_c + 2 * st_r;
+#pragma unroll
+  for (int e = 0; e < 2; ++e) {
+    const int d = d0 + e;
+    unsigned w01 = e ? (((unsigned)dw[0] >> 16) | ((unsigned)dw[1] & 0xffff0000u))
+                     : (((unsigned)dw[0] & 0xffffu) | ((unsigned)dw[1] << 16));
+    unsigned w23 = e ? (((unsigned)dw[2] >> 16) | ((unsigned)dw[3] & 0xffff0000u))
+                     : (((unsigned)dw[2] & 0xffffu) | ((unsigned)dw[3] << 16));
+    int2v_t pair = {(int)w01, (int)w23};
+    *reinterpret_cast<int2v_t*>(img + tt_swz(d, rq)) = pair;
+  }
+}
+
+__device__ __forceinline__ void tt_store(const char* img, short* __restrict__ out,
+                                         int64_t R, int r0, int c0) {
+  const int tid = threadIdx.x;
+#pragma unroll
+  for (int pass = 0; pass < 4; ++pass) {
+    const int d = 32 * pass + (tid >> 3);
+    const int p = tid & 7;
+    const bf16x8_t v = *reinterpret_cast<const bf16x8_t*>(img + tt_swz(d, 8 * p));
+    *reinterpret_cast<bf16x8_t*>(out + (int64_t)(c0 + d) * R + r0 + 8 * p) = v;
+  }
+}
+
+}
diff --git a/lpp_amd/ops/linear.py b/lpp_amd/ops/linear.py
--- a/lpp_amd/ops/linear.py
+++ b/lpp_amd/ops/linear.py
@@ -32,6 +32,54 @@
 
 
 _xt_cache = _XTCache()
+
+
+class _HandoffCache:
+
+    CAPACITY = 4
+    __slots__ = ("entries", "hits", "misses")
+
+    def __init__(self):
+        self.entries = []
+        self.hits = 0
+        self.misses = 0
+
+    def put(self, natural: torch.Tensor, image: torch.Tensor) -> None:
+        self.entries.append((natural, image))
+        if len(self.entries) > self.CAPACITY:
+            del self.entries[0]
+
+    def take(self, dy2: torch.Tensor):
+        for i, (nat, img) in enumerate(self.entries):
+            if (nat.data_ptr() == dy2.data_ptr() and nat.shape == dy2.shape
+                    and nat.dtype == dy2.dtype):
+                del self.entries[i]
+                self.hits += 1
+                return img
+        self.misses += 1
+        return None
+
+    def clear(self):
+        self.entries.clear()
+
+    def __len__(self):
+        return len(self.entries)
+
+
+_handoff = _HandoffCache()
+
+
+def bwd_handoff_enabled() -> bool:
+    return os.environ.get("LPP_BWD_HANDOFF", "1") == "1"
+
+
+def register_handoff(natural: torch.Tensor, image: torch.Tensor) -> None:
+    _handoff.put(natural.view(image.shape[1], image.shape[0]), image)
+
+
+def clear_backward_caches() -> None:
+    _xt_cache.clear()
+    _handoff.clear()
 
 
 def _wgrad_pre_enabled() -> bool:
@@ -80,7 +128,9 @@
         dy2 = dy.reshape(-1, dy.shape[-1])
         if _wgrad_pre_enabled():
             xT = _xt_cache.get(ext, x2)
-            dyT = ext.transpose2d(dy2)
+            dyT = _handoff.take(dy2) if bwd_handoff_enabled() else None
+            if dyT is None:
+                dyT = ext.transpose2d(dy2)
             if _wgrad_bf16d_enabled():
                 ext.accum_bf16_f32(ctx.main_grad.view(-1),
                                    torch.matmul(dyT, xT.t()).view(-1))
diff --git a/lpp_amd/ops/rmsnorm.py b/lpp_amd/ops/rmsnorm.py
--- a/lpp_amd/ops/rmsnorm.py
+++ b/lpp_amd/ops/rmsnorm.py
@@ -4,6 +4,7 @@
 import torch
 
 from . import use_hip, extension
+from .linear import bwd_handoff_enabled, register_handoff
 
 
 def rmsnorm_ref(x: torch.Tensor, weight: torch.Tensor, eps: float) -> torch.Tensor:
@@ -32,3 +33,39 @@
     if use_hip(x):
         return _RMSNormHIP.apply(x.contiguous(), weight, eps)
     return rmsnorm_ref(x, weight, eps)
+
+
+class _RMSNormForkHIP(torch.autograd.Function):
+
+    @staticmethod
+    def forward(ctx, x, weight, eps, n, want_t):
+        ext = extension()
+        y, invrms = ext.rmsnorm_fwd(x, weight, eps)
+        ctx.save_for_backward(x, weight, invrms)
+        ctx.want_t = want_t
+        ctx.set_materialize_grads(False)
+        return (x.view_as(x),) + tuple(y.view_as(y) for _ in range(n))
+
+    @staticmethod
+    def backward(ctx, dres, *dys):
+        x, weight, invrms = ctx.saved_tensors
+        ext = extension()
+        parts = [d.contiguous() for d in reversed(dys) if d is not None]
+        if not parts:
+            return dres, None, None, None, None
+        dx, dw, dxT = ext.rmsnorm_bwd_fused(
+            parts, x, weight, invrms,
+            dres.contiguous() if dres is not None else None, ctx.want_t)
+        if dxT.numel():
+            register_handoff(dx, dxT)
+        return dx, dw, None, None, None
+
+
+def rmsnorm_fork(x: torch.Tensor, weight: torch.Tensor, eps: float, n: int,
+                 want_t: bool = True):
+    return _RMSNormForkHIP.apply(x.contiguous(), weight, eps, n, want_t)
+
+
+def rmsnorm_fork_applies(x: torch.Tensor) -> bool:
+    return (use_hip(x) and torch.is_grad_enabled() and x.dtype is torch.bfloat16
+            and bwd_handoff_enabled())
diff --git a/lpp_amd/ops/rope.py b/lpp_amd/ops/rope.py
--- a/lpp_amd/ops/rope.py
+++ b/lpp_amd/ops/rope.py
@@ -6,6 +6,7 @@
 import torch
 
 from . import use_hip, extension
+from .linear import bwd_handoff_enabled, register_handoff
 
 _CACHE: dict = {}
 
@@ -52,8 +53,13 @@
     def backward(ctx, dy):
         cos, sin = ctx.saved_tensors
         ext = extension()
-        dx = ext.rope_bwd(dy.contiguous(), cos, sin, ctx.pos_offset)
-        return dx, None, None, None
+        if not bwd_handoff_enabled():
+            dx = ext.rope_bwd(dy.contiguous(), cos, sin, ctx.pos_offset)
+            return dx, None, None, None
+        out = ext.rope_bwd_t(dy.contiguous(), cos, sin, ctx.pos_offset)
+        if len(out) == 2:
+            register_handoff(out[0], out[1])
+        return out[0], None, None, None
 
 
 def apply_rope(
diff --git a/lpp_amd/ops/swiglu.py b/lpp_amd/ops/swiglu.py
--- a/lpp_amd/ops/swiglu.py
+++ b/lpp_amd/ops/swiglu.py
@@ -4,6 +4,7 @@
 import torch
 
 from . import use_hip, extension
+from .linear import bwd_handoff_enabled, register_handoff
 
 
 def swiglu_ref(gate: torch.Tensor, up: torch.Tensor) -> torch.Tensor:
@@ -23,8 +24,14 @@
     def backward(ctx, dy):
         gate, up = ctx.saved_tensors
         ext = extension()
-        dgate, dup = ext.swiglu_bwd(dy.contiguous(), gate, up)
-        return dgate, dup
+        if not bwd_handoff_enabled():
+            dgate, dup = ext.swiglu_bwd(dy.contiguous(), gate, up)
+            return dgate, dup
+        out = ext.swiglu_bwd_t(dy.contiguous(), gate, up)
+        if len(out) == 4:
+            register_handoff(out[0], out[2])
+            register_handoff(out[1], out[3])
+        return out[0], out[1]
 
 
 def swiglu(gate: torch.Tensor, up: torch.Tensor) -> torch.Tensor:
```

Result: faster. 24350 tokens/s, median of 6 (+1.7%).
